# W-Ted/F3D-Gaus

Hardware: AMD Instinct MI355X
Metric: rendered views/sec at 256x256 (N Gaussians, K cams) (higher is better)
Workload: dtype f32; 1 GPU; C2: 1 image/GPU, 196608 Gaussians (sigma0=0.01), 120-view orbit @256x256, GOF forward raster only; timed region = render + 8-bit RGB frames copied to pinned host memory; compositing arithmetic: fast = error-free float32 pairs for the float64 island + hardware exp/rcp/rsq; every channel within 1e-4 of the oracle (RGB <= 3e-7), EXCEPT that the distortion channel (values 1e-7..1e-5 from cancelling fl; gaussians=196608, views=120, resolution=256, tile_cull=1, views_per_call=120, render_mode=fast, channels=all, parallelism=single GPU

## Files before the change

f3d-gaus_amd/csrc/f3dg_api.hip:

```cpp
#include "f3dg_common.h"

#include <stdio.h>
#include <string.h>
#include <time.h>
#include <mutex>
#include <vector>

namespace {

thread_local char g_last_error[512] = "";

size_t align_up(size_t x, size_t a) { return (x + a - 1) / a * a; }

__global__ void init_header_kernel(F3dgHeader* hdr, unsigned capacity, unsigned alpha_fast = 0, unsigned save_aux = 0)
{
    if (threadIdx.x < 64) {
        unsigned* w = reinterpret_cast<unsigned*>(hdr);
        w[threadIdx.x] = 0;
    }
    __syncthreads();
    if (threadIdx.x == 0) { hdr->capacity = capacity; hdr->alpha_fast = alpha_fast; hdr->save_aux = save_aux; }
}

__global__ void fill_background_kernel(int V, size_t HW, const float* __restrict__ bg, int bg_per_view,
                                       float* __restrict__ out)
{
    const size_t n = (size_t)V * F3DG_OUT_CHANNELS * HW;
    for (size_t i = (size_t)blockIdx.x * blockDim.x + threadIdx.x; i < n; i += (size_t)gridDim.x * blockDim.x)
        out[i] = 0.0f;
    (void)bg; (void)bg_per_view;
}

__global__ void export_ids_kernel(const unsigned* __restrict__ src, size_t n, unsigned* __restrict__ dst)
{
    for (size_t i = (size_t)blockIdx.x * blockDim.x + threadIdx.x; i < n; i += (size_t)gridDim.x * blockDim.x)
        dst[i] = src[i] & F3DG_ID_MASK;
}

enum { ST_PREPROCESS = 0, ST_BINNING, ST_RENDER, ST_COUNT };
enum { BW_RENDER = 0, BW_GAUSSIAN, BW_COUNT };
struct ProfCall { hipEvent_t ev[ST_COUNT + 1]; };
struct ProfBwd { hipEvent_t ev[BW_COUNT + 1]; };
struct Prof {
    bool enabled = false;
    std::vector<ProfCall> calls;
    std::vector<ProfCall> pool;
    std::vector<ProfBwd> bwd;
};
thread_local Prof g_prof;

ProfCall* prof_begin(hipStream_t s)
{
    if (!g_prof.enabled) return nullptr;
    ProfCall c;
    if (!g_prof.pool.empty()) { c = g_prof.pool.back(); g_prof.pool.pop_back(); }
    else for (int i = 0; i <= ST_COUNT; i++) if (hipEventCreate(&c.ev[i]) != hipSuccess) return nullptr;
    g_prof.calls.push_back(c);
    (void)hipEventRecord(c.ev[0], s);
    return &g_prof.calls.back();
}
inline void prof_mark(ProfCall* c, int stage_done, hipStream_t s) { if (c) (void)hipEventRecord(c->ev[stage_done + 1], s); }

}

int f3dg_prof_bwd_begin(hipStream_t s)
{
    if (!g_prof.enabled) return -1;
    ProfBwd b;
    for (int i = 0; i <= BW_COUNT; i++) if (hipEventCreate(&b.ev[i]) != hipSuccess) return -1;
    g_prof.bwd.push_back(b);
    (void)hipEventRecord(b.ev[0], s);
    return (int)g_prof.bwd.size() - 1;
}
void f3dg_prof_bwd_mark(int slot, int stage_done, hipStream_t s)
{
    if (slot >= 0 && slot < (int)g_prof.bwd.size()) (void)hipEventRecord(g_prof.bwd[slot].ev[stage_done + 1], s);
}

int g_f3dg_small_path = 1;
int g_f3dg_small_path_aux = 1;
namespace {
struct SmallShape { unsigned v[4]; };
std::vector<SmallShape> g_small_disabled;
std::mutex g_small_mutex, g_sites_mutex;
bool small_disabled(unsigned P, unsigned V, unsigned W, unsigned H)
{
    std::lock_guard<std::mutex> lock(g_small_mutex);
    for (const SmallShape& d : g_small_disabled)
        if (d.v[0] == P && d.v[1] == V && d.v[2] == W && d.v[3] == H) return true;
    return false;
}
void small_disable(unsigned P, unsigned V, unsigned W, unsigned H)
{
    std::lock_guard<std::mutex> lock(g_small_mutex);
    for (const SmallShape& d : g_small_disabled)
        if (d.v[0] == P && d.v[1] == V && d.v[2] == W && d.v[3] == H) return;
    g_small_disabled.push_back({{P, V, W, H}});
}
}
std::atomic<unsigned long long> g_f3dg_kernel_launches{0};
int g_f3dg_render_fast = 1;
int g_f3dg_render_pack = -1;
int g_f3dg_render_count = 0;
int g_f3dg_render_lowocc = 1;
#define F3DG_RENDER_UNROLL_DEFAULT -1
#define F3DG_RENDER_SPLIT_DEFAULT -1
int g_f3dg_render_split = F3DG_RENDER_SPLIT_DEFAULT;
int g_f3dg_render_unroll = F3DG_RENDER_UNROLL_DEFAULT;
int g_f3dg_bwd_occ = 5;
int g_f3dg_tile_cull = 1;
int g_f3dg_reference_kernels = 0;

extern "C" int f3dg_set_option(const char* name, int value)
{
    if (!name) return F3DG_ERR_BAD_ARG;
    if (strcmp(name, "render_fast") == 0) { g_f3dg_render_fast = value < 0 ? 0 : value > 2 ? 2 : value; return F3DG_OK; }
    if (strcmp(name, "tile_cull") == 0) { g_f3dg_tile_cull = value != 0; return F3DG_OK; }
    if (strcmp(name, "small_path") == 0) { g_f3dg_small_path = value != 0; if (value == 2) { std::lock_guard<std::mutex> lock(g_small_mutex); g_small_disabled.clear(); } return F3DG_OK; }
    if (strcmp(name, "small_path_aux") == 0) { g_f3dg_small_path_aux = value != 0; return F3DG_OK; }
    if (strcmp(name, "render_pack") == 0) { g_f3dg_render_pack = value < 0 ? -1 : value != 0; return F3DG_OK; }
    if (strcmp(name, "render_pack_th") == 0) { g_f3dg_render_pack_th = value < 0 ? 0 : value > 64 ? 64 : value; return F3DG_OK; }
    if (strcmp(name, "render_scan") == 0) { g_f3dg_render_scan = value < 0 ? -1 : value != 0; return F3DG_OK; }
    if (strcmp(name, "render_scan_min") == 0) { g_f3dg_render_scan_min = value < 0 ? 0 : value > 64 ? 64 : value; return F3DG_OK; }
    if (strcmp(name, "render_scan_th") == 0) { g_f3dg_render_scan_th = value < 0 ? 0 : value > 64 ? 64 : value; return F3DG_OK; }
    if (strcmp(name, "render_lowocc") == 0) { g_f3dg_render_lowocc = value < 0 ? 1 : value > 64 ? 64 : value; return F3DG_OK; }
    if (strcmp(name, "render_unroll") == 0) { g_f3dg_render_unroll = value < 0 ? F3DG_RENDER_UNROLL_DEFAULT : value < 1 ? 1 : value > 2 ? 2 : value; return F3DG_OK; }
    if (strcmp(name, "bwd_dense") == 0) { g_f3dg_bwd_dense = value != 0; return F3DG_OK; }
    if (strcmp(name, "bwd_occ") == 0) { g_f3dg_bwd_occ = (value >= 2 && value <= 6) ? value : 5; return F3DG_OK; }
    if (strcmp(name, "render_count") == 0) { g_f3dg_render_count = value != 0; return F3DG_OK; }
    if (strcmp(name, "time_launches") == 0) { g_f3dg_time_launches = value != 0; return F3DG_OK; }
    if (strcmp(name, "reference_kernels") == 0) { g_f3dg_reference_kernels = value != 0; return F3DG_OK; }
    if (strcmp(name, "render_split") == 0) { g_f3dg_render_split = value < 1 ? F3DG_RENDER_SPLIT_DEFAULT : value > 3 ? 3 : value; return F3DG_OK; }
    return F3DG_ERR_BAD_ARG;
}

int g_f3dg_time_launches = 0;
namespace { struct LaunchSite { const char* file; int line; long long ns, n, max_ns; }; std::vector<LaunchSite> g_sites; }
long long f3dg_now_ns()
{
    timespec ts;
    clock_gettime(CLOCK_MONOTONIC, &ts);
    return (long long)ts.tv_sec * 1000000000ll + ts.tv_nsec;
}
void f3dg_note_launch_time(const char* file, int line, long long ns)
{
    std::lock_guard<std::mutex> lock(g_sites_mutex);
    for (LaunchSite& s : g_sites)
        if (s.file == file && s.line == line) { s.ns += ns; s.n++; if (ns > s.max_ns) s.max_ns = ns; return; }
    g_sites.push_back({file, line, ns, 1, ns});
}
extern "C" int f3dg_debug_launch_times(int reset)
{
    std::lock_guard<std::mutex> lock(g_sites_mutex);
    for (const LaunchSite& s : g_sites) {
        const char* base = strrchr(s.file, '/');
        fprintf(stderr, "%-22s:%4d  %6lld launches  %8.2f us avg  %9.1f us max\n", base ? base + 1 : s.file, s.line, s.n,
                1e-3 * (double)s.ns / (double)s.n, 1e-3 * (double)s.max_ns);
    }
    if (reset) g_sites.clear();
    return F3DG_OK;
}

extern "C" long long f3dg_debug_launch_count(int reset)
{
    return (long long)(reset ? g_f3dg_kernel_launches.exchange(0ull) : g_f3dg_kernel_launches.load());
}

extern "C" int f3dg_profile_enable(int on)
{
    g_prof.enabled = on != 0;
    return F3DG_OK;
}

extern "C" int f3dg_profile_collect(double* h_stage_ms, int* h_calls) { return f3dg_profile_collect_calls(h_stage_ms, h_calls, nullptr, 0); }

extern "C" int f3dg_profile_collect_calls(double* h_stage_ms, int* h_calls, double* h_per_call, int max_calls)
{
    double sum[ST_COUNT] = { 0, 0, 0 };
    int k = 0;
    for (ProfCall& c : g_prof.calls) {
        F3DG_HIP_CHECK(hipEventSynchronize(c.ev[ST_COUNT]));
        for (int i = 0; i < ST_COUNT; i++) {
            float ms = 0;
            F3DG_HIP_CHECK(hipEventElapsedTime(&ms, c.ev[i], c.ev[i + 1]));
            sum[i] += ms;
            if (h_per_call && k < max_calls) h_per_call[3 * k + i] = ms;
        }
        k++;
        g_prof.pool.push_back(c);
    }
    double bsum[BW_COUNT] = { 0, 0 };
    for (ProfBwd& b : g_prof.bwd) {
        F3DG_HIP_CHECK(hipEventSynchronize(b.ev[BW_COUNT]));
        for (int i = 0; i < BW_COUNT; i++) {
            float ms = 0;
            F3DG_HIP_CHECK(hipEventElapsedTime(&ms, b.ev[i], b.ev[i + 1]));
            bsum[i] += ms;
        }
        for (int i = 0; i <= BW_COUNT; i++) (void)hipEventDestroy(b.ev[i]);
    }
    g_prof.bwd.clear();
    if (h_calls) *h_calls = (int)g_prof.calls.size();
    g_prof.calls.clear();
    if (h_stage_ms) {
        for (int i = 0; i < ST_COUNT; i++) h_stage_ms[i] = sum[i];
        for (int i = 0; i < BW_COUNT; i++) h_stage_ms[ST_COUNT + i] = bsum[i];
    }
    return F3DG_OK;
}

int f3dg_set_hip_error(hipError_t e, const char* where)
{
    snprintf(g_last_error, sizeof g_last_error, "%s: %s", where, hipGetErrorString(e));
    return F3DG_ERR_HIP;
}

extern "C" const char* f3dg_version(void) { return "f3dg-hip gfx950 0.2.0"; }
extern "C" const char* f3dg_last_error(void) { return g_last_error; }

int f3dg_sort_passes(int V, int T);

F3dgLayout f3dg_layout(int P, int W, int H, int V, long long cap)
{
    F3dgLayout L;
    memset(&L, 0, sizeof L);
    const size_t VP = (size_t)V * (size_t)(P > 0 ? P : 1);
    const size_t HW = (size_t)W * H;
    const size_t T = (size_t)((W + F3DG_TILE - 1) / F3DG_TILE) * ((H + F3DG_TILE - 1) / F3DG_TILE);
    const size_t C = (size_t)(cap > 0 ? cap : 1);
    L.sort_blocks = (unsigned)((C + F3DG_SORT_CHUNK - 1) / F3DG_SORT_CHUNK);
    const size_t scan_a = (VP + F3DG_SCAN_CHUNK - 1) / F3DG_SCAN_CHUNK;
    const size_t gsort_blocks = (size_t)V * (((size_t)(P > 0 ? P : 1) + F3DG_SORT_CHUNK - 1) / F3DG_SORT_CHUNK);
    const size_t tile_blocks = (size_t)L.sort_blocks + (size_t)V;
    const size_t hist_blocks = gsort_blocks > tile_blocks ? gsort_blocks : tile_blocks;
    const size_t scan_b = ((size_t)256 * hist_blocks + F3DG_SCAN_CHUNK - 1) / F3DG_SCAN_CHUNK;
    L.scan_tmp_elems = (unsigned)((scan_a > scan_b ? scan_a : scan_b) + 1);

    size_t off = 0;
    auto take = [&](size_t bytes) { size_t o = off; off = align_up(off + bytes, 256); return o; };
    L.header = take(sizeof(F3dgHeader));
    L.rec = take(VP * sizeof(F3dgRec));
    L.means2D = take(VP * sizeof(float2));
    L.bbox = take(VP * sizeof(float4));
    L.cull = take(VP * sizeof(float4));
    L.depths = take(VP * sizeof(float));
    L.conic = take(VP * sizeof(float4));
    L.radii = take(VP * sizeof(int));
    L.tiles = take(VP * sizeof(unsigned));
    L.offsets = take(VP * sizeof(unsigned));
    L.clamped = take(VP);
    L.rects = take(VP * sizeof(uint2));
    L.gsort = take(4 * VP * sizeof(unsigned));
    L.scan_tmp = take((size_t)L.scan_tmp_elems * sizeof(unsigned));
    L.keys[0] = take(C * 8);
    L.keys[1] = take(C * 4);
    L.vals[0] = take(C * 4);
    L.vals[1] = take(C * 4);
    L.segtab_minmax = (unsigned)((size_t)2 * (V + 1) + (size_t)8 * (V / 8 + 2));
    L.segtab = take(((size_t)L.segtab_minmax + (size_t)2 * V + 2 * gsort_blocks) * sizeof(unsigned));
    L.hist = take((size_t)256 * hist_blocks * sizeof(unsigned));
    L.ranges = take((size_t)V * T * sizeof(uint2));
    L.final_T = take((size_t)V * 4 * HW * sizeof(float));
    L.n_contrib = take((size_t)V * 2 * HW * sizeof(unsigned));
    L.bwd_acc = take(VP * 16 * sizeof(double));
    L.small_cap = f3dg_small_shape(P, W, H, V) ? (unsigned)F3DG_SMALL_CAP : 0u;
    L.small_boxes = take(L.small_cap ? (size_t)V * ((P + 63) / 64) * sizeof(uint2) : 0);
    L.small_cnt = take((size_t)V * T * sizeof(unsigned));
    L.small_list = take((size_t)V * T * L.small_cap * sizeof(unsigned));
    L.total = off;
    return L;
}

extern "C" size_t f3dg_workspace_bytes(int P, int W, int H, int n_views, long long max_rendered)
{
    if (P < 0 || W <= 0 || H <= 0 || n_views <= 0 || max_rendered < 0) return 0;
    return f3dg_layout(P, W, H, n_views, max_rendered).total;
}

namespace {

int check_gaussian_args(int P, int D, int M, const float* means3D, const float* shs, const float* colors_precomp,
                        const float* opacities, const float* scales, const float* rotations, const float* cov3D_precomp,
                        const float* view2gaussian_precomp, const float* viewmatrix, const float* projmatrix,
                        const float* cam_pos)
{
    (void)P;
    if (!means3D || !opacities || !viewmatrix || !projmatrix || !cam_pos) return F3DG_ERR_BAD_ARG;
    if ((shs == nullptr) == (colors_precomp == nullptr)) return F3DG_ERR_BAD_ARG;
    const bool have_sr = scales != nullptr && rotations != nullptr;
    if (have_sr == (cov3D_precomp != nullptr)) return F3DG_ERR_BAD_ARG;
    if (!have_sr && view2gaussian_precomp == nullptr) return F3DG_ERR_BAD_ARG;
    if (shs && (M <= 0 || D < 0 || D > 3 || (D + 1) * (D + 1) > M)) return F3DG_ERR_BAD_ARG;
    return F3DG_OK;
}

int run_geometry(hipStream_t s, char* ws, const F3dgLayout& L, int n_views, int views_per_set, int P, int D, int M, int W, int H,
                 const float* means3D, const float* shs, const float* colors_precomp, const float* opacities,
                 const float* scales, float scale_modifier, const float* rotations, const float* cov3D_precomp,
                 const float* view2gaussian_precomp, const float* viewmatrix, const float* projmatrix,
                 const float* cam_pos, float tan_fovx, float tan_fovy, float focal_x, float focal_y, float kernel_size,
                 int* radii_used, int save_aux, int need_box, int tile_cull, ProfCall* prof, F3dgHeaderInit init, int small = 0)
{
    int rc = f3dg_launch_preprocess(s, n_views, views_per_set, P, D, M, means3D, scales, scale_modifier, rotations, opacities, shs,
                                    cov3D_precomp, colors_precomp, view2gaussian_precomp, viewmatrix, projmatrix,
                                    cam_pos, W, H, tan_fovx, tan_fovy, focal_x, focal_y, kernel_size,
                                    reinterpret_cast<F3dgRec*>(ws + L.rec), reinterpret_cast<float2*>(ws + L.means2D),
                                    reinterpret_cast<float*>(ws + L.depths), reinterpret_cast<unsigned*>(ws + L.gsort),
                                    reinterpret_cast<uint2*>(ws + L.rects),
                                    need_box ? reinterpret_cast<float4*>(ws + L.bbox) : nullptr,
                                    reinterpret_cast<float4*>(ws + L.cull),
                                    reinterpret_cast<float4*>(ws + L.conic), radii_used,
                                    reinterpret_cast<unsigned*>(ws + L.tiles),
                                    reinterpret_cast<unsigned char*>(ws + L.clamped), save_aux, tile_cull, init,
                                    small ? reinterpret_cast<uint2*>(ws + L.small_boxes) : nullptr);
    if (rc != F3DG_OK) return rc;
    prof_mark(prof, ST_PREPROCESS, s);
    rc = small ? f3dg_launch_small_bin(s, n_views, P, W, H, L, ws) : f3dg_launch_binning(s, n_views, P, W, H, L, ws, save_aux);
    if (rc != F3DG_OK) return rc;
    prof_mark(prof, ST_BINNING, s);
    return F3DG_OK;
}

}

extern "C" int f3dg_forward_batched(void* stream, void* workspace, size_t workspace_bytes, long long max_rendered,
                                    int n_views, int P, int D, int M,
                                    const float* background, int W, int H,
                                    const float* means3D, const float* shs, const float* colors_precomp,
                                    const float* opacities, const float* scales, float scale_modifier,
                                    const float* rotations, const float* cov3D_precomp,
                                    const float* view2gaussian_precomp,
                                    const float* viewmatrix, const float* projmatrix, const float* cam_pos,
                                    float tan_fovx, float tan_fovy, float kernel_size,
                                    float* out_color, int* radii, unsigned flags)
{
    return f3dg_forward_sets(stream, workspace, workspace_bytes, max_rendered, 1, n_views, P, D, M, background, W, H, means3D, shs,
                             colors_precomp, opacities, scales, scale_modifier, rotations, cov3D_precomp, view2gaussian_precomp,
                             viewmatrix, projmatrix, cam_pos, tan_fovx, tan_fovy, kernel_size, out_color, radii, flags);
}

extern "C" int f3dg_forward_sets(void* stream, void* workspace, size_t workspace_bytes, long long max_rendered,
                                 int n_sets, int views_per_set, int P, int D, int M,
                                 const float* background, int W, int H,
                                 const float* means3D, const float* shs, const float* colors_precomp,
                                 const float* opacities, const float* scales, float scale_modifier,
                                 const float* rotations, const float* cov3D_precomp,
                                 const float* view2gaussian_precomp,
                                 const float* viewmatrix, const float* projmatrix, const float* cam_pos,
                                 float tan_fovx, float tan_fovy, float kernel_size,
                                 float* out_color, int* radii, unsigned flags)
{
    if (n_sets <= 0 || views_per_set <= 0 || (long long)n_sets * views_per_set > 0x7FFFFFF0ll) return F3DG_ERR_BAD_ARG;
    const int n_views = n_sets * views_per_set;
    hipStream_t s = (hipStream_t)stream;
    if (n_views <= 0 || P < 0 || W <= 0 || H <= 0 || max_rendered < 0 || !out_color || !background || !workspace)
        return F3DG_ERR_BAD_ARG;
    if (max_rendered > 0xFFFFFFF0ll || (long long)n_views * P > 0xFFFFFFF0ll || P > (int)F3DG_ID_MASK)
        return F3DG_ERR_BAD_ARG;
    const F3dgLayout L = f3dg_layout(P, W, H, n_views, max_rendered);
    if (workspace_bytes < L.total) return F3DG_ERR_WORKSPACE;
    char* ws = static_cast<char*>(workspace);
    F3dgHeader* hdr = reinterpret_cast<F3dgHeader*>(ws + L.header);
    const size_t HW = (size_t)W * H;

    const int save_aux = (flags & F3DG_FLAG_SAVE_AUX) ? 1 : 0;
    if ((flags & F3DG_FLAG_SETS_AUX) && !save_aux) return F3DG_ERR_BAD_ARG;
    if (n_sets > 1 && ((save_aux && !(flags & F3DG_FLAG_SETS_AUX)) || view2gaussian_precomp != nullptr)) return F3DG_ERR_BAD_ARG;
    const int fast = g_f3dg_reference_kernels || (flags & F3DG_FLAG_EXACT) ? 0 : (flags & F3DG_FLAG_FAST) ? 1 : f3dg_render_uses_fast(save_aux);
    const int tile_cull = (flags & F3DG_FLAG_NO_TILE_CULL) ? 0 : g_f3dg_tile_cull;
    const int small = g_f3dg_small_path && !(flags & F3DG_FLAG_NO_SMALL_PATH) && (!save_aux || g_f3dg_small_path_aux) && n_sets == 1 && P > 0 && L.small_cap != 0 &&
                      !g_f3dg_reference_kernels && !small_disabled((unsigned)P, (unsigned)n_views, (unsigned)W, (unsigned)H);
    const F3dgHeaderInit hinit = { hdr, (unsigned)max_rendered, (unsigned)fast, (unsigned)save_aux, (unsigned)small,
                                   { (unsigned)P, (unsigned)n_views, (unsigned)W, (unsigned)H } };
    if (P == 0)
        F3DG_KLAUNCH(init_header_kernel, dim3(1), dim3(64), 0, s, hdr, (unsigned)max_rendered, (unsigned)fast, (unsigned)save_aux);

    if (P == 0) {
        F3DG_KLAUNCH(fill_background_kernel, dim3(1024), dim3(256), 0, s, n_views, HW, background,
                           (flags & F3DG_FLAG_BG_PER_VIEW) ? 1 : 0, out_color);
        F3DG_HIP_CHECK(hipGetLastError());
        return F3DG_OK;
    }
    int rc = check_gaussian_args(P, D, M, means3D, shs, colors_precomp, opacities, scales, rotations, cov3D_precomp,
                                 view2gaussian_precomp, viewmatrix, projmatrix, cam_pos);
    if (rc != F3DG_OK) return rc;

    const float focal_y = H / (2.0f * tan_fovy);
    const float focal_x = W / (2.0f * tan_fovx);
    int* radii_used = radii ? radii : reinterpret_cast<int*>(ws + L.radii);

    ProfCall* prof = prof_begin(s);
    rc = run_geometry(s, ws, L, n_views, views_per_set, P, D, M, W, H, means3D, shs, colors_precomp, opacities, scales, scale_modifier,
                      rotations, cov3D_precomp, view2gaussian_precomp, viewmatrix, projmatrix, cam_pos, tan_fovx,
                      tan_fovy, focal_x, focal_y, kernel_size, radii_used, save_aux,
                      save_aux , tile_cull, prof, hinit, small);
    if (rc != F3DG_OK) return rc;

    rc = f3dg_launch_render(s, n_views, P, W, H, focal_x, focal_y, hdr,
                              reinterpret_cast<const uint2*>(ws + L.ranges),
                              reinterpret_cast<const unsigned*>(ws + (small ? L.small_list : L.vals[0])),
                              reinterpret_cast<const F3dgRec*>(ws + L.rec),
                              reinterpret_cast<const float4*>(ws + L.cull), background,
                              (flags & F3DG_FLAG_BG_PER_VIEW) ? 1 : 0, out_color,
                              reinterpret_cast<float*>(ws + L.final_T),
                              reinterpret_cast<unsigned*>(ws + L.n_contrib), save_aux,
                              flags & (F3DG_FLAG_SKIP_NORMAL | F3DG_FLAG_SKIP_DISTORTION), fast, (flags & F3DG_FLAG_SCAN) ? 1 : 0);
    prof_mark(prof, ST_RENDER, s);
    return rc;
}

extern "C" size_t f3dg_integrate_workspace_bytes(int P, int PN, int W, int H, long long max_rendered)
{
    if (P < 0 || PN < 0 || W <= 0 || H <= 0 || max_rendered < 0) return 0;
    return f3dg_integ_layout(P, PN, W, H, max_rendered).total;
}

extern "C" size_t f3dg_integrate_workspace_bytes_batched(int P, int PN, int W, int H, int n_views, long long max_rendered)
{
    if (P < 0 || PN < 0 || W <= 0 || H <= 0 || n_views <= 0 || max_rendered < 0) return 0;
    return f3dg_integ_layout(P, PN, W, H, max_rendered, n_views).total;
}

extern "C" long long f3dg_integrate_prepare_batched(void* stream, void* workspace, size_t workspace_bytes, long long max_rendered,
                                                    int n_views, int PN_max, int P, int D, int M, const float* background, int W, int H,
                                                    const float* means3D, const float* shs, const float* colors_precomp,
                                                    const float* opacities, const float* scales, float scale_modifier,
                                                    const float* rotations, const float* cov3D_precomp,
                                                    const float* view2gaussian_precomp, const float* viewmatrix,
                                                    const float* projmatrix, const float* cam_pos, float tan_fovx, float tan_fovy,
                                                    float kernel_size, float* out_color, int* radii, long long* h_needed)
{
    hipStream_t s = (hipStream_t)stream;
    if (n_views <= 0 || PN_max < 0 || P <= 0 || W <= 0 || H <= 0 || max_rendered < 0 || !out_color || !workspace || !background)
        return F3DG_ERR_BAD_ARG;
    if (max_rendered > 0xFFFFFFF0ll || (long long)n_views * P > 0xFFFFFFF0ll || P > (int)F3DG_ID_MASK) return F3DG_ERR_BAD_ARG;
    const F3dgLayout L = f3dg_layout(P, W, H, n_views, max_rendered);
    const F3dgIntegLayout I = f3dg_integ_layout(P, PN_max, W, H, max_rendered, n_views);
    if (workspace_bytes < I.total) return F3DG_ERR_WORKSPACE;
    char* ws = static_cast<char*>(workspace);
    F3dgHeader* hdr = reinterpret_cast<F3dgHeader*>(ws + L.header);
    if (h_needed) *h_needed = 0;
    const F3dgHeaderInit hinit = { hdr, (unsigned)max_rendered, 0u, 0u, 0u, { (unsigned)P, (unsigned)n_views, (unsigned)W, (unsigned)H } };
    int rc = check_gaussian_args(P, D, M, means3D, shs, colors_precomp, opacities, scales, rotations, cov3D_precomp,
                                 view2gaussian_precomp, viewmatrix, projmatrix, cam_pos);
    if (rc != F3DG_OK) return rc;
    const float focal_y = H / (2.0f * tan_fovy);
    const float focal_x = W / (2.0f * tan_fovx);
    int* radii_used = radii ? radii : reinterpret_cast<int*>(ws + L.radii);
    rc = run_geometry(s, ws, L, n_views, n_views, P, D, M, W, H, means3D, shs, colors_precomp, opacities, scales, scale_modifier,
                      rotations, cov3D_precomp, view2gaussian_precomp, viewmatrix, projmatrix, cam_pos, tan_fovx,
                      tan_fovy, focal_x, focal_y, kernel_size, radii_used, 0, 1 ,
                      0 , nullptr, hinit);
    if (rc != F3DG_OK) return rc;
    rc = f3dg_launch_integrate_pass1(s, n_views, P, W, H, focal_x, focal_y, L, I, ws, background, out_color);
    if (rc != F3DG_OK) return rc;
    long long n = 0;
    rc = f3dg_read_status(stream, workspace, &n);
    if (h_needed) *h_needed = n;
    if (rc != F3DG_OK) return rc;
    return n;
}

extern "C" long long f3dg_integrate_prepare(void* stream, void* workspace, size_t workspace_bytes, long long max_rendered,
                                            int PN_max, int P, int D, int M, const float* background, int W, int H,
                                            const float* means3D, const float* shs, const float* colors_precomp,
                                            const float* opacities, const float* scales, float scale_modifier,
                                            const float* rotations, const float* cov3D_precomp,
                                            const float* view2gaussian_precomp, const float* viewmatrix,
                                            const float* projmatrix, const float* cam_pos, float tan_fovx, float tan_fovy,
                                            float kernel_size, float* out_color, int* radii, long long* h_needed)
{
    return f3dg_integrate_prepare_batched(stream, workspace, workspace_bytes, max_rendered, 1, PN_max, P, D, M, background, W, H, means3D,
                                          shs, colors_precomp, opacities, scales, scale_modifier, rotations, cov3D_precomp,
                                          view2gaussian_precomp, viewmatrix, projmatrix, cam_pos, tan_fovx, tan_fovy, kernel_size,
                                          out_color, radii, h_needed);
}

extern "C" int f3dg_integrate_points_view(void* stream, void* workspace, size_t workspace_bytes, long long max_rendered,
                                          int n_views, int view, int PN, int P, int W, int H, const float* points3D,
                                          const float* viewmatrix, float tan_fovx, float tan_fovy, float* out_color,
                                          float* out_alpha_integrated, float* out_color_integrated, float* alpha_min)
{
    hipStream_t s = (hipStream_t)stream;
    if (PN < 0 || P <= 0 || W <= 0 || H <= 0 || max_rendered < 0 || !out_color || !workspace || !viewmatrix || n_views <= 0 ||
        view < 0 || view >= n_views)
        return F3DG_ERR_BAD_ARG;
    if (PN == 0) return F3DG_OK;
    if (!points3D) return F3DG_ERR_BAD_ARG;
    const F3dgLayout L = f3dg_layout(P, W, H, n_views, max_rendered);
    const F3dgIntegLayout I = f3dg_integ_layout(P, PN, W, H, max_rendered, n_views);
    if (workspace_bytes < I.total) return F3DG_ERR_WORKSPACE;
    const float focal_y = H / (2.0f * tan_fovy);
    const float focal_x = W / (2.0f * tan_fovx);
    return f3dg_launch_integrate_points(s, view, P, PN, W, H, focal_x, focal_y, L, I, static_cast<char*>(workspace), points3D,
                                        viewmatrix, out_color, out_alpha_integrated, out_color_integrated, alpha_min);
}

extern "C" int f3dg_debug_integrate_redo(void* stream, const void* workspace, int P, int PN_max, int W, int H, int n_views,
                                         long long max_rendered, int* h_tiles)
{
    if (!workspace || !h_tiles || P <= 0 || W <= 0 || H <= 0 || n_views <= 0 || PN_max < 0 || max_rendered < 0) return F3DG_ERR_BAD_ARG;
    const F3dgIntegLayout I = f3dg_integ_layout(P, PN_max, W, H, max_rendered, n_views);
    const size_t T = (size_t)((W + F3DG_TILE - 1) / F3DG_TILE) * ((H + F3DG_TILE - 1) / F3DG_TILE);
    std::vector<unsigned> flags((size_t)n_views * T);
    F3DG_HIP_CHECK(hipMemcpyAsync(flags.data(), static_cast<const char*>(workspace) + I.redo, flags.size() * sizeof(unsigned),
                                  hipMemcpyDeviceToHost, (hipStream_t)stream));
    F3DG_HIP_CHECK(hipStreamSynchronize((hipStream_t)stream));
    int n = 0;
    for (unsigned f : flags) n += f != 0u;
    *h_tiles = n;
    return F3DG_OK;
}

extern "C" int f3dg_integrate_points(void* stream, void* workspace, size_t workspace_bytes, long long max_rendered,
                                     int PN, int P, int W, int H, const float* points3D, const float* viewmatrix,
                                     float tan_fovx, float tan_fovy, float* out_color, float* out_alpha_integrated,
                                     float* out_color_integrated, float* alpha_min)
{
    return f3dg_integrate_points_view(stream, workspace, workspace_bytes, max_rendered, 1, 0, PN, P, W, H, points3D, viewmatrix, tan_fovx,
                                      tan_fovy, out_color, out_alpha_integrated, out_color_integrated, alpha_min);
}

extern "C" long long f3dg_integrate(void* stream, void* workspace, size_t workspace_bytes, long long max_rendered,
                                    int PN, int P, int D, int M, const float* background, int W, int H,
                                    const float* points3D, const float* means3D, const float* shs,
                                    const float* colors_precomp, const float* opacities, const float* scales,
                                    float scale_modifier, const float* rotations, const float* cov3D_precomp,
                                    const float* view2gaussian_precomp, const float* viewmatrix,
                                    const float* projmatrix, const float* cam_pos, float tan_fovx, float tan_fovy,
                                    float kernel_size, const float* subpixel_offset, int prefiltered,
                                    float* out_color, int* radii, float* out_alpha_integrated,
                                    float* out_color_integrated, long long* h_needed)
{
    (void)subpixel_offset;
    (void)prefiltered;
    hipStream_t s = (hipStream_t)stream;
    if (PN < 0 || P < 0 || W <= 0 || H <= 0 || max_rendered < 0 || !out_color || !workspace) return F3DG_ERR_BAD_ARG;
    if (PN > 0 && (!points3D || !out_alpha_integrated || !out_color_integrated)) return F3DG_ERR_BAD_ARG;
    if (h_needed) *h_needed = 0;
    if (P == 0 || PN == 0) {
        if (workspace_bytes < sizeof(F3dgHeader)) return F3DG_ERR_WORKSPACE;
        F3DG_KLAUNCH(init_header_kernel, dim3(1), dim3(64), 0, s, reinterpret_cast<F3dgHeader*>(workspace), (unsigned)max_rendered);
        int rc = f3dg_launch_integrate_fill(s, W, H, PN, out_color, out_alpha_integrated, out_color_integrated);
        if (rc != F3DG_OK) return rc;
        F3DG_HIP_CHECK(hipStreamSynchronize(s));
        return 0;
    }
    const long long n = f3dg_integrate_prepare(stream, workspace, workspace_bytes, max_rendered, PN, P, D, M, background, W, H,
                                               means3D, shs, colors_precomp, opacities, scales, scale_modifier, rotations,
                                               cov3D_precomp, view2gaussian_precomp, viewmatrix, projmatrix, cam_pos,
                                               tan_fovx, tan_fovy, kernel_size, out_color, radii, h_needed);
    if (n < 0) return n;
    const int rc = f3dg_integrate_points(stream, workspace, workspace_bytes, max_rendered, PN, P, W, H, points3D, viewmatrix,
                                         tan_fovx, tan_fovy, out_color, out_alpha_integrated, out_color_integrated, nullptr);
    if (rc != F3DG_OK) return rc;
    return n;
}

extern "C" int f3dg_read_status(void* stream, const void* workspace, long long* h_num_rendered)
{
    if (!workspace) return F3DG_ERR_BAD_ARG;
    F3dgHeader h;
    F3DG_HIP_CHECK(hipMemcpyAsync(&h, workspace, sizeof h, hipMemcpyDeviceToHost, (hipStream_t)stream));
    F3DG_HIP_CHECK(hipStreamSynchronize((hipStream_t)stream));
    if (h_num_rendered) *h_num_rendered = (long long)h.num_rendered;
    if (h.small_overflow) small_disable(h.small_shape[0], h.small_shape[1], h.small_shape[2], h.small_shape[3]);
    return h.overflow ? F3DG_ERR_OVERFLOW : F3DG_OK;
}

namespace {
struct StatusSlot { F3dgHeader* host; hipEvent_t ev; bool busy; };
std::vector<StatusSlot> g_status;
std::mutex g_status_mutex;
int finish_status(const F3dgHeader& h, long long* h_num_rendered)
{
    if (h_num_rendered) *h_num_rendered = (long long)h.num_rendered;
    if (h.small_overflow) small_disable(h.small_shape[0], h.small_shape[1], h.small_shape[2], h.small_shape[3]);
    return h.overflow ? F3DG_ERR_OVERFLOW : F3DG_OK;
}
}

extern "C" int f3dg_status_post(void* stream, const void* workspace)
{
    if (!workspace) return F3DG_ERR_BAD_ARG;
    int ticket = -1;
    StatusSlot sl = { nullptr, nullptr, false };
    {
        std::lock_guard<std::mutex> lock(g_status_mutex);
        for (size_t i = 0; i < g_status.size(); i++)
            if (!g_status[i].busy) { ticket = (int)i; break; }
        if (ticket < 0) {
            StatusSlot fresh = { nullptr, nullptr, false };
            F3DG_HIP_CHECK(hipHostMalloc(reinterpret_cast<void**>(&fresh.host), sizeof(F3dgHeader), hipHostMallocDefault));
            const hipError_t e = hipEventCreateWithFlags(&fresh.ev, hipEventDisableTiming);
            if (e != hipSuccess) { (void)hipHostFree(fresh.host); return f3dg_set_hip_error(e, "hipEventCreateWithFlags"); }
            g_status.push_back(fresh);
            ticket = (int)g_status.size() - 1;
        }
        g_status[ticket].busy = true;
        sl = g_status[ticket];
    }
    hipError_t e = hipMemcpyAsync(sl.host, workspace, sizeof(F3dgHeader), hipMemcpyDeviceToHost, (hipStream_t)stream);
    if (e == hipSuccess) e = hipEventRecord(sl.ev, (hipStream_t)stream);
    if (e != hipSuccess) {
        std::lock_guard<std::mutex> lock(g_status_mutex);
        g_status[ticket].busy = false;
        return f3dg_set_hip_error(e, "f3dg_status_post");
    }
    return ticket;
}

extern "C" int f3dg_status_poll(int ticket, int wait, long long* h_num_rendered)
{
    StatusSlot sl;
    {
        std::lock_guard<std::mutex> lock(g_status_mutex);
        if (ticket < 0 || ticket >= (int)g_status.size() || !g_status[ticket].busy) return F3DG_ERR_BAD_ARG;
        sl = g_status[ticket];
    }
    if (wait) F3DG_HIP_CHECK(hipEventSynchronize(sl.ev));
    else {
        const hipError_t q = hipEventQuery(sl.ev);
        if (q == hipErrorNotReady) return F3DG_PENDING;
        F3DG_HIP_CHECK(q);
    }
    const int rc = finish_status(*sl.host, h_num_rendered);
    std::lock_guard<std::mutex> lock(g_status_mutex);
    g_status[ticket].busy = false;
    return rc;
}

extern "C" int f3dg_backward_pairs(void* stream, const void* workspace, long long* h_pairs)
{
    if (!workspace || !h_pairs) return F3DG_ERR_BAD_ARG;
    F3dgHeader h;
    F3DG_HIP_CHECK(hipMemcpyAsync(&h, workspace, sizeof h, hipMemcpyDeviceToHost, (hipStream_t)stream));
    F3DG_HIP_CHECK(hipStreamSynchronize((hipStream_t)stream));
    *h_pairs = (long long)h.bwd_pairs;
    return h.bwd_stale ? F3DG_ERR_STATE : F3DG_OK;
}

extern "C" long long f3dg_forward(void* stream, void* workspace, size_t workspace_bytes, long long max_rendered,
                                  int P, int D, int M, const float* background, int W, int H,
                                  const float* means3D, const float* shs, const float* colors_precomp,
                                  const float* opacities, const float* scales, float scale_modifier,
                                  const float* rotations, const float* cov3D_precomp,
                                  const float* view2gaussian_precomp,
                                  const float* viewmatrix, const float* projmatrix, const float* cam_pos,
                                  float tan_fovx, float tan_fovy, float kernel_size, int prefiltered,
                                  float* out_color, int* radii, unsigned flags, long long* h_needed)
{
    (void)prefiltered;
    int rc = f3dg_forward_batched(stream, workspace, workspace_bytes, max_rendered, 1, P, D, M, background, W, H,
                                  means3D, shs, colors_precomp, opacities, scales, scale_modifier, rotations,
                                  cov3D_precomp, view2gaussian_precomp, viewmatrix, projmatrix, cam_pos, tan_fovx,
                                  tan_fovy, kernel_size, out_color, radii, flags & ~F3DG_FLAG_BG_PER_VIEW);
    if (rc != F3DG_OK) return rc;
    long long n = 0;
    rc = f3dg_read_status(stream, workspace, &n);
    if (h_needed) *h_needed = n;
    if (rc != F3DG_OK) return rc;
    return n;
}

extern "C" int f3dg_debug_export(void* stream, const void* workspace, int P, int W, int H, int n_views,
                                 long long max_rendered, float* rec , float* means2D ,
                                 float* conic , unsigned* tiles , unsigned* offsets ,
                                 unsigned char* clamped , unsigned long long* keys_sorted ,
                                 unsigned* point_list , unsigned* ranges ,
                                 float* final_T , unsigned* n_contrib , float* depths )
{
    hipStream_t s = (hipStream_t)stream;
    if (!workspace) return F3DG_ERR_BAD_ARG;
    const F3dgLayout L = f3dg_layout(P, W, H, n_views, max_rendered);
    const char* ws = static_cast<const char*>(workspace);
    const size_t VP = (size_t)n_views * P, HW = (size_t)W * H;
    F3dgHeader h;
    F3DG_HIP_CHECK(hipMemcpyAsync(&h, ws + L.header, sizeof h, hipMemcpyDeviceToHost, s));
    F3DG_HIP_CHECK(hipStreamSynchronize(s));
    if ((means2D || conic || tiles || offsets || clamped || keys_sorted || final_T || n_contrib || depths) && !h.save_aux)
        return F3DG_ERR_BAD_ARG;
    if (h.small_path) {
        if (h.overflow) return F3DG_ERR_OVERFLOW;
        if (offsets || keys_sorted) return F3DG_ERR_STATE;
        const int rcs = f3dg_launch_small_export(s, n_views, W, H, L, ws, point_list, ranges);
        if (rcs != F3DG_OK) return rcs;
        point_list = nullptr;
        ranges = nullptr;
    }
    const size_t T = (size_t)((W + F3DG_TILE - 1) / F3DG_TILE) * ((H + F3DG_TILE - 1) / F3DG_TILE);
    const size_t C = (size_t)max_rendered;
    if (keys_sorted && P > 0) {
        const int rck = f3dg_launch_export_keys(s, n_views, P, W, H, L, const_cast<char*>(ws));
        if (rck != F3DG_OK) return rck;
    }
#define CP(dst, off, bytes) if (dst && (bytes)) F3DG_HIP_CHECK(hipMemcpyAsync(dst, ws + (off), (bytes), hipMemcpyDeviceToDevice, s))
    CP(rec, L.rec, VP * sizeof(F3dgRec));
    CP(means2D, L.means2D, VP * 8);
    CP(conic, L.conic, VP * 16);
    CP(tiles, L.tiles, VP * 4);
    CP(offsets, L.offsets, VP * 4);
    CP(clamped, L.clamped, VP);
    CP(keys_sorted, L.keys[0], C * 8);
    if (point_list && C)
        F3DG_KLAUNCH(export_ids_kernel, dim3((unsigned)((C + 1023) / 1024 < 4096 ? (C + 1023) / 1024 : 4096)), dim3(256), 0, s,
                           reinterpret_cast<const unsigned*>(ws + L.vals[0]), C, point_list);
    CP(ranges, L.ranges, (size_t)n_views * T * 8);
    CP(final_T, L.final_T, (size_t)n_views * 4 * HW * 4);
    CP(n_contrib, L.n_contrib, (size_t)n_views * 2 * HW * 4);
    CP(depths, L.depths, VP * 4);
#undef CP
    return F3DG_OK;
}
```

f3d-gaus_amd/csrc/f3dg_binning.hip:

```cpp
#include "f3dg_common.h"

namespace {

typedef unsigned long long u64;
typedef unsigned int u32;

__global__ void __launch_bounds__(F3DG_BLOCK)
scan_reduce_kernel(const u32* __restrict__ in, u64 n, u32* __restrict__ block_sums)
{
    __shared__ u32 wsum[F3DG_BLOCK / 64];
    const u64 base = (u64)blockIdx.x * F3DG_SCAN_CHUNK;
    u32 s = 0;
#pragma unroll
    for (int i = 0; i < F3DG_SCAN_ITEMS; i++) {
        const u64 k = base + (u64)i * F3DG_BLOCK + threadIdx.x;
        if (k < n) s += in[k];
    }
#pragma unroll
    for (int off = 32; off > 0; off >>= 1) s += __shfl_down(s, off, 64);
    if ((threadIdx.x & 63) == 0) wsum[threadIdx.x >> 6] = s;
    __syncthreads();
    if (threadIdx.x == 0) block_sums[blockIdx.x] = wsum[0] + wsum[1] + wsum[2] + wsum[3];
}

__global__ void __launch_bounds__(1024)
scan_blocksums_kernel(u32* __restrict__ block_sums, u32 nblocks, F3dgHeader* __restrict__ hdr)
{
    __shared__ u32 wtot[16];
    __shared__ u32 carry_s;
    __shared__ u64 carry64_s, wtot64[16];
    if (threadIdx.x == 0) { carry_s = 0; carry64_s = 0; }
    __syncthreads();
    const int lane = threadIdx.x & 63, wave = threadIdx.x >> 6;
    for (u32 start = 0; start < nblocks; start += 1024) {
        const u32 i = start + threadIdx.x;
        const u32 v = i < nblocks ? block_sums[i] : 0;
        u32 x = v;
#pragma unroll
        for (int off = 1; off < 64; off <<= 1) {
            const u32 y = __shfl_up(x, off, 64);
            if (lane >= off) x += y;
        }
        if (lane == 63) wtot[wave] = x;
        unsigned long long v64 = v;
#pragma unroll
        for (int off = 32; off > 0; off >>= 1) v64 += __shfl_down(v64, off, 64);
        if (lane == 0) wtot64[wave] = v64;
        __syncthreads();
        u32 wave_off = 0;
        for (int w = 0; w < wave; w++) wave_off += wtot[w];
        const u32 carry = carry_s;
        if (i < nblocks) block_sums[i] = carry + wave_off + x - v;
        __syncthreads();
        if (threadIdx.x == 1023) {
            carry_s = carry + wave_off + x;
            u64 t = 0;
            for (int w = 0; w < 16; w++) t += wtot64[w];
            carry64_s += t;
        }
        __syncthreads();
    }
    if (hdr && threadIdx.x == 0) {
        const u64 total = carry64_s;
        hdr->num_rendered = total > 0xFFFFFFFFull ? 0xFFFFFFFFu : (u32)total;
        hdr->overflow = total > (u64)hdr->capacity ? 1u : 0u;
    }
}

__global__ void __launch_bounds__(F3DG_BLOCK)
scan_apply_kernel(const u32* in, u32* out , u64 n, const u32* __restrict__ block_sums,
                  int exclusive)
{
    __shared__ u32 wtot[F3DG_BLOCK / 64];
    const u64 base = (u64)blockIdx.x * F3DG_SCAN_CHUNK + (u64)threadIdx.x * F3DG_SCAN_ITEMS;
    u32 v[F3DG_SCAN_ITEMS];
    u32 s = 0;
    if (base + F3DG_SCAN_ITEMS <= n) {
#pragma unroll
        for (int i = 0; i < F3DG_SCAN_ITEMS / 4; i++) {
            const uint4 w = reinterpret_cast<const uint4*>(in + base)[i];
            v[4 * i] = w.x; v[4 * i + 1] = w.y; v[4 * i + 2] = w.z; v[4 * i + 3] = w.w;
        }
    } else {
#pragma unroll
        for (int i = 0; i < F3DG_SCAN_ITEMS; i++) v[i] = (base + i < n) ? in[base + i] : 0;
    }
#pragma unroll
    for (int i = 0; i < F3DG_SCAN_ITEMS; i++) s += v[i];
    const int lane = threadIdx.x & 63, wave = threadIdx.x >> 6;
    u32 x = s;
#pragma unroll
    for (int off = 1; off < 64; off <<= 1) {
        const u32 y = __shfl_up(x, off, 64);
        if (lane >= off) x += y;
    }
    if (lane == 63) wtot[wave] = x;
    __syncthreads();
    u32 run = block_sums[blockIdx.x] + x - s;
    for (int w = 0; w < wave; w++) run += wtot[w];
    u32 o[F3DG_SCAN_ITEMS];
#pragma unroll
    for (int i = 0; i < F3DG_SCAN_ITEMS; i++) {
        const u32 before = run;
        run += v[i];
        o[i] = exclusive ? before : run;
    }
    if (base + F3DG_SCAN_ITEMS <= n) {
#pragma unroll
        for (int i = 0; i < F3DG_SCAN_ITEMS / 4; i++)
            reinterpret_cast<uint4*>(out + base)[i] = make_uint4(o[4 * i], o[4 * i + 1], o[4 * i + 2], o[4 * i + 3]);
    } else {
#pragma unroll
        for (int i = 0; i < F3DG_SCAN_ITEMS; i++)
            if (base + i < n) out[base + i] = o[i];
    }
}


struct SegChunk {
    u64 seg_base;
    u64 obase;
    u32 n;
    u32 cps;
    u32 c;
    u32 seg;
};

struct SegTable {
    const u32* vstart;
    const u32* bglob;
    const u32* xprefix;
    u32 xstride;
    u32 V;
};

struct ShiftDigit {
    int shift;
    u32 mask = 255u;
    __device__ __forceinline__ u32 operator()(u32 k) const { return (k >> shift) & mask; }
};
struct CompactDigit {
    u32 kbase;
    __device__ __forceinline__ u32 operator()(u32 k) const { const u32 d = (k - kbase) >> 16; return d < 255u ? d : 255u; }
};

template <typename K, typename DIGIT, bool MINMAX = false>
__device__ __forceinline__ void hist_chunk(const K* __restrict__ keys, const SegChunk& ck, const DIGIT digit, u32* __restrict__ hist,
                                           u32 (*h)[256], u32* __restrict__ minmax = nullptr)
{
    u32 kmin = 0xFFFFFFFFu, kmax = 0u;
#pragma unroll
    for (int w = 0; w < F3DG_BLOCK / 64; w++) h[w][threadIdx.x] = 0;
    __syncthreads();
    u32* hw = h[threadIdx.x >> 6];
    constexpr int VEC = 16 / (int)sizeof(K);
    typedef K __attribute__((ext_vector_type(VEC))) KV;
    const u64 base = (u64)ck.c * F3DG_SORT_CHUNK;
    const u64 g0 = ck.seg_base + base;
    const u64 g1 = ck.seg_base + ((u64)ck.n - base < (u64)F3DG_SORT_CHUNK ? (u64)ck.n : base + F3DG_SORT_CHUNK);
    for (u64 a = (g0 & ~(u64)(VEC - 1)) + (u64)threadIdx.x * VEC; a < g1; a += (u64)F3DG_BLOCK * VEC) {
        const KV w = *reinterpret_cast<const KV*>(keys + a);
#pragma unroll
        for (int q = 0; q < VEC; q++) {
            if (a + q >= g0 && a + q < g1) {
                const u32 key = (u32)w[q];
                atomicAdd(&hw[digit(key)], 1u);
                if (MINMAX && key != 0xFFFFFFFFu) { kmin = key < kmin ? key : kmin; kmax = key > kmax ? key : kmax; }
            }
        }
    }
    __shared__ u32 wmm[2][F3DG_BLOCK / 64];
    if (MINMAX) {
#pragma unroll
        for (int off = 32; off > 0; off >>= 1) {
            const u32 a = __shfl_down(kmin, off, 64), b = __shfl_down(kmax, off, 64);
            kmin = a < kmin ? a : kmin; kmax = b > kmax ? b : kmax;
        }
        if ((threadIdx.x & 63) == 0) { wmm[0][threadIdx.x >> 6] = kmin; wmm[1][threadIdx.x >> 6] = kmax; }
    }
    __syncthreads();
    if (MINMAX && threadIdx.x == 0) {
        u32 a = wmm[0][0], b = wmm[1][0];
#pragma unroll
        for (int w = 1; w < F3DG_BLOCK / 64; w++) { a = wmm[0][w] < a ? wmm[0][w] : a; b = wmm[1][w] > b ? wmm[1][w] : b; }
        minmax[0] = a; minmax[1] = b;
    }
    hist[ck.obase + (u64)threadIdx.x * ck.cps + ck.c] = h[0][threadIdx.x] + h[1][threadIdx.x] + h[2][threadIdx.x] + h[3][threadIdx.x];
}

struct ScatterShared {
    u32 cnt[F3DG_BLOCK / 64][256];
    u32 lbase[256];
    u32 gdelta[256];
    u32 wtot[F3DG_BLOCK / 64];
    u32 sval[F3DG_SORT_CHUNK];
};

template <typename K, bool IOTA, typename DIGIT>
__device__ __forceinline__ void scatter_chunk(const K* __restrict__ keys_in, const u32* __restrict__ vals_in, K* __restrict__ keys_out,
                                              u32* __restrict__ vals_out, const SegChunk& ck, const DIGIT digit,
                                              const u32* __restrict__ offsets , ScatterShared& sh, K* skey)
{
    const u32 n = ck.n;
    const u64 block_base = (u64)ck.c * F3DG_SORT_CHUNK;
    const u32 in_block = (u32)((n - block_base) < (u64)F3DG_SORT_CHUNK ? (n - block_base) : (u64)F3DG_SORT_CHUNK);
    const int lane = threadIdx.x & 63, wave = threadIdx.x >> 6;
#pragma unroll
    for (int w = 0; w < F3DG_BLOCK / 64; w++) sh.cnt[w][threadIdx.x] = 0;
    __syncthreads();

    const u64 wave_base = block_base + (u64)wave * (64 * F3DG_SORT_ITEMS);
    u32 key[F3DG_SORT_ITEMS];
    u32 val[F3DG_SORT_ITEMS];
    u32 rank[F3DG_SORT_ITEMS];
    const u64 lane_lt = ((u64)1 << lane) - 1;
#pragma unroll
    for (int r = 0; r < F3DG_SORT_ITEMS; r++) {
        const u64 i = wave_base + (u64)r * 64 + lane;
        const bool valid = i < n;
        key[r] = valid ? (u32)keys_in[ck.seg_base + i] : 0u;
        val[r] = IOTA ? (u32)i : (valid ? vals_in[ck.seg_base + i] : 0u);
    }
#pragma unroll
    for (int r = 0; r < F3DG_SORT_ITEMS; r++) {
        const u64 i = wave_base + (u64)r * 64 + lane;
        const bool valid = i < n;
        const u32 d = digit(key[r]);
        u64 diff = 0;
#pragma unroll
        for (int b = 0; b < 8; b++) {
            const u32 own = (u32)((int)(d << (31 - b)) >> 31);
            const u64 bal = __ballot(own != 0u);
            diff |= bal ^ (((u64)own << 32) | own);
        }
        const u64 same = __ballot(valid) & ~diff;
        const u32 below = (u32)__popcll(same & lane_lt);
        const u32 prev = sh.cnt[wave][d];
        rank[r] = prev + below;
        __builtin_amdgcn_wave_barrier();
        if (valid && below == 0) sh.cnt[wave][d] = prev + (u32)__popcll(same);
        __builtin_amdgcn_wave_barrier();
    }
    __syncthreads();
    {
        const u32 d = threadIdx.x;
        const u32 c0 = sh.cnt[0][d], c1 = sh.cnt[1][d], c2 = sh.cnt[2][d], c3 = sh.cnt[3][d];
        const u32 tot = c0 + c1 + c2 + c3;
        u32 x = tot;
#pragma unroll
        for (int off = 1; off < 64; off <<= 1) {
            const u32 y = __shfl_up(x, off, 64);
            if (lane >= off) x += y;
        }
        if (lane == 63) sh.wtot[wave] = x;
        __syncthreads();
        u32 excl = x - tot;
        for (int w = 0; w < wave; w++) excl += sh.wtot[w];
        sh.lbase[d] = excl;
        sh.gdelta[d] = offsets[ck.obase + (u64)d * ck.cps + ck.c] - excl;
        sh.cnt[0][d] = excl;
        sh.cnt[1][d] = excl + c0;
        sh.cnt[2][d] = excl + c0 + c1;
        sh.cnt[3][d] = excl + c0 + c1 + c2;
    }
    __syncthreads();
#pragma unroll
    for (int r = 0; r < F3DG_SORT_ITEMS; r++) {
        const u64 i = wave_base + (u64)r * 64 + lane;
        if (i < n) {
            const u32 d = digit(key[r]);
            const u32 slot = sh.cnt[wave][d] + rank[r];
            skey[slot] = (K)key[r];
            sh.sval[slot] = val[r];
        }
    }
    __syncthreads();
    for (u32 slot = threadIdx.x; slot < in_block; slot += F3DG_BLOCK) {
        const K k = skey[slot];
        const u32 d = digit((u32)k);
        const u32 pos = sh.gdelta[d] + slot;
        if (keys_out) keys_out[pos] = k;
        vals_out[pos] = sh.sval[slot];
    }
}

__device__ __forceinline__ SegChunk fixed_chunk(u32 seg_len, u32 cps)
{
    u32 seg, c;
    f3dg_xcd_map(blockIdx.x, gridDim.x / cps, cps, seg, c);
    SegChunk ck;
    ck.seg_base = (u64)seg * seg_len; ck.obase = (u64)seg * 256u * cps; ck.n = seg_len; ck.cps = cps; ck.c = c; ck.seg = seg;
    return ck;
}

__device__ __forceinline__ bool gsort_compact(const u32* __restrict__ minmax, u32 view, u32& kbase)
{
    const u32 kmin = minmax[2 * view], kmax = minmax[2 * view + 1];
    kbase = kmin & 0xFFFF0000u;
    return kmin <= kmax && ((kmax - kbase) >> 24) == 0u;
}

template <int PASS>
__global__ void __launch_bounds__(F3DG_BLOCK)
gsort_hist_kernel(const u32* __restrict__ keys, u32 seg_len, u32 cps, u32* __restrict__ hist, const u32* __restrict__ minmax,
                  u32* __restrict__ chunk_minmax)
{
    __shared__ u32 h[F3DG_BLOCK / 64][256];
    const SegChunk ck = fixed_chunk(seg_len, cps);
    if constexpr (PASS == 0) {
        hist_chunk<u32, ShiftDigit>(keys, ck, ShiftDigit{0}, hist, h);
    } else if constexpr (PASS == 1) {
        hist_chunk<u32, ShiftDigit, true>(keys, ck, ShiftDigit{8}, hist, h, chunk_minmax + 2 * ((size_t)ck.seg * cps + ck.c));
    } else {
        u32 kbase;
        const bool compact = gsort_compact(minmax, ck.seg, kbase);
        if (!compact) {
            hist_chunk<u32, ShiftDigit>(keys, ck, ShiftDigit{8 * PASS}, hist, h);
        } else if constexpr (PASS == 2) {
            hist_chunk<u32, CompactDigit>(keys, ck, CompactDigit{kbase}, hist, h);
        } else {
            const u64 base = (u64)ck.c * F3DG_SORT_CHUNK;
            const u32 in_chunk = (u32)((ck.n - base) < (u64)F3DG_SORT_CHUNK ? (ck.n - base) : (u64)F3DG_SORT_CHUNK);
            hist[ck.obase + (u64)threadIdx.x * ck.cps + ck.c] = threadIdx.x == 0 ? in_chunk : 0u;
        }
    }
}

__global__ void __launch_bounds__(1024)
gsort_scan_kernel(u32 n_per_seg , u32 seg_len, u32* __restrict__ hist)
{
    __shared__ u32 wtot[16];
    __shared__ u32 carry_s;
    u32* h = hist + (size_t)blockIdx.x * n_per_seg;
    const u32 lane = threadIdx.x & 63u, wave = threadIdx.x >> 6;
    if (threadIdx.x == 0) carry_s = blockIdx.x * seg_len;
    __syncthreads();
    for (u32 base = 0; base < n_per_seg; base += 4096u) {
        const u32 i = base + 4u * threadIdx.x;
        uint4 v = make_uint4(0u, 0u, 0u, 0u);
        if (i < n_per_seg) v = *reinterpret_cast<const uint4*>(h + i);
        const u32 tot = v.x + v.y + v.z + v.w;
        u32 x = tot;
#pragma unroll
        for (int off = 1; off < 64; off <<= 1) {
            const u32 y = __shfl_up(x, off, 64);
            if (lane >= (u32)off) x += y;
        }
        if (lane == 63u) wtot[wave] = x;
        __syncthreads();
        u32 before = carry_s + x - tot;
        for (u32 w = 0; w < wave; w++) before += wtot[w];
        if (i < n_per_seg)
            *reinterpret_cast<uint4*>(h + i) = make_uint4(before, before + v.x, before + v.x + v.y, before + v.x + v.y + v.z);
        __syncthreads();
        if (threadIdx.x == 1023u) carry_s = before + tot;
        __syncthreads();
    }
}

__global__ void __launch_bounds__(64)
gsort_range_kernel(u32 cps, const u32* __restrict__ chunk_minmax, u32* __restrict__ minmax)
{
    u32 kmin = 0xFFFFFFFFu, kmax = 0u;
    for (u32 c = threadIdx.x; c < cps; c += 64) {
        const u32 a = chunk_minmax[2 * ((size_t)blockIdx.x * cps + c)], b = chunk_minmax[2 * ((size_t)blockIdx.x * cps + c) + 1];
        kmin = a < kmin ? a : kmin; kmax = b > kmax ? b : kmax;
    }
#pragma unroll
    for (int off = 32; off > 0; off >>= 1) {
        const u32 a = __shfl_down(kmin, off, 64), b = __shfl_down(kmax, off, 64);
        kmin = a < kmin ? a : kmin; kmax = b > kmax ? b : kmax;
    }
    if (threadIdx.x == 0) { minmax[2 * blockIdx.x] = kmin; minmax[2 * blockIdx.x + 1] = kmax; }
}

template <int PASS>
__global__ void __launch_bounds__(F3DG_BLOCK)
gsort_scatter_kernel(const u32* __restrict__ keys_in, const u32* __restrict__ vals_in, u32* __restrict__ keys_out,
                     u32* __restrict__ vals_out, u32 seg_len, u32 cps, const u32* __restrict__ offsets, const u32* __restrict__ minmax)
{
    __shared__ ScatterShared sh;
    __shared__ u32 skey[F3DG_SORT_CHUNK];
    const SegChunk ck = fixed_chunk(seg_len, cps);
    if constexpr (PASS == 0) {
        scatter_chunk<u32, true, ShiftDigit>(keys_in, vals_in, keys_out, vals_out, ck, ShiftDigit{0}, offsets, sh, skey);
    } else if constexpr (PASS == 1) {
        scatter_chunk<u32, false, ShiftDigit>(keys_in, vals_in, keys_out, vals_out, ck, ShiftDigit{8}, offsets, sh, skey);
    } else {
        u32 kbase;
        const bool compact = gsort_compact(minmax, ck.seg, kbase);
        if (!compact)
            scatter_chunk<u32, false, ShiftDigit>(keys_in, vals_in, PASS == 3 ? (u32*)nullptr : keys_out, vals_out, ck, ShiftDigit{8 * PASS}, offsets, sh, skey);
        else if constexpr (PASS == 2)
            scatter_chunk<u32, false, CompactDigit>(keys_in, vals_in, (u32*)nullptr, vals_out, ck, CompactDigit{kbase}, offsets, sh, skey);
    }
}

__global__ void __launch_bounds__(512)
view_segments_kernel(int V, int P, const u32* __restrict__ offsets_sorted, const F3dgHeader* __restrict__ hdr, u32* __restrict__ vstart,
                     u32* __restrict__ bglob, u32* __restrict__ xprefix, u32 xstride)
{
    __shared__ u32 carry;
    __shared__ u32 wtot[8];
    const u32 lane = threadIdx.x & 63u, wave = threadIdx.x >> 6;
    const bool dead = hdr->overflow != 0;
    auto start_of = [&](u32 v) -> u32 {
        const u64 i = (u64)v * (u64)P;
        return (dead || i == 0) ? 0u : offsets_sorted[i - 1];
    };
    auto chunks_of = [&](u32 v) -> u32 {
        const u32 n = start_of(v + 1) - start_of(v);
        return (n + F3DG_SORT_CHUNK - 1) / F3DG_SORT_CHUNK;
    };
    if (threadIdx.x == 0) carry = 0;
    __syncthreads();
    for (u32 v0 = 0; v0 < (u32)V; v0 += 512) {
        const u32 v = v0 + threadIdx.x;
        const u32 c = v < (u32)V ? chunks_of(v) : 0u;
        u32 x = c;
#pragma unroll
        for (int off = 1; off < 64; off <<= 1) {
            const u32 y = __shfl_up(x, off, 64);
            if (lane >= (u32)off) x += y;
        }
        if (lane == 63) wtot[wave] = x;
        __syncthreads();
        u32 woff = carry;
        for (u32 w = 0; w < wave; w++) woff += wtot[w];
        if (v < (u32)V) { vstart[v] = start_of(v); bglob[v] = woff + x - c; }
        __syncthreads();
        if (threadIdx.x == 511) carry = woff + x;
        __syncthreads();
    }
    if (threadIdx.x == 0) { vstart[V] = start_of((u32)V); bglob[V] = carry; }
    const u32 nk = ((u32)V > wave) ? ((u32)V - wave + 7u) / 8u : 0u;
    u32 run = 0;
    for (u32 k0 = 0; k0 < nk; k0 += 64) {
        const u32 k = k0 + lane;
        const u32 c = k < nk ? chunks_of(wave + 8u * k) : 0u;
        u32 x = c;
#pragma unroll
        for (int off = 1; off < 64; off <<= 1) {
            const u32 y = __shfl_up(x, off, 64);
            if (lane >= (u32)off) x += y;
        }
        if (k < nk) xprefix[wave * xstride + k] = run + x - c;
        run += __shfl(x, 63, 64);
    }
    if (lane == 0) xprefix[wave * xstride + nk] = run;
}

__global__ void __launch_bounds__(F3DG_BLOCK)
ranges_from_offsets_kernel(u32 V, u32 T, int tile_bits, const u32* __restrict__ bglob, const u32* __restrict__ offsets,
                           const F3dgHeader* __restrict__ hdr, uint2* __restrict__ ranges)
{
    const u32 i = blockIdx.x * F3DG_BLOCK + threadIdx.x;
    if (i >= V * T) return;
    const u32 v = i / T, t = i % T;
    const u32 b0 = bglob[v], cpv = bglob[v + 1] - b0;
    uint2 r = make_uint2(0u, 0u);
    if (cpv != 0u && !hdr->overflow) {
        const u32 d = ((v << tile_bits) | t) & 255u;
        const u32 lo = offsets[256ull * b0 + (u64)d * cpv], hi = offsets[256ull * b0 + (u64)(d + 1u) * cpv];
        if (hi > lo) r = make_uint2(lo, hi);
    }
    ranges[i] = r;
}

__device__ __forceinline__ bool var_chunk(const SegTable& st, u32 f, u32& k, SegChunk& ck)
{
    const u32 x = blockIdx.x & 7u;
    const u32* xp = st.xprefix + x * st.xstride;
    const u32 nk = (st.V > x) ? (st.V - x + 7u) / 8u : 0u;
    while (k < nk && f >= xp[k + 1]) k++;
    if (k >= nk) return false;
    const u32 v = x + 8u * k;
    const u32 s0 = st.vstart[v], b0 = st.bglob[v];
    ck.seg_base = s0; ck.n = st.vstart[v + 1] - s0; ck.cps = st.bglob[v + 1] - b0; ck.obase = 256ull * b0; ck.c = f - xp[k];
    return true;
}

template <typename K>
__global__ void __launch_bounds__(F3DG_BLOCK)
radix2_hist_var_kernel(const K* __restrict__ keys, SegTable st, int shift, u32 mask, u32* __restrict__ hist)
{
    __shared__ u32 h[F3DG_BLOCK / 64][256];
    u32 k = 0;
    SegChunk ck;
    for (u32 f = blockIdx.x >> 3; var_chunk(st, f, k, ck); f += gridDim.x >> 3)
        hist_chunk<K, ShiftDigit>(keys, ck, ShiftDigit{shift, mask}, hist, h);
}

template <typename K>
__global__ void __launch_bounds__(F3DG_BLOCK)
radix2_scatter_var_kernel(const K* __restrict__ keys_in, const u32* __restrict__ vals_in, K* __restrict__ keys_out,
                          u32* __restrict__ vals_out, SegTable st, int shift, u32 mask, const u32* __restrict__ offsets)
{
    __shared__ ScatterShared sh;
    __shared__ K skey[F3DG_SORT_CHUNK];
    u32 k = 0;
    SegChunk ck;
    for (u32 f = blockIdx.x >> 3; var_chunk(st, f, k, ck); f += gridDim.x >> 3) {
        scatter_chunk<K, false, ShiftDigit>(keys_in, vals_in, keys_out, vals_out, ck, ShiftDigit{shift, mask}, offsets, sh, skey);
        __syncthreads();
    }
}

__global__ void __launch_bounds__(F3DG_BLOCK)
gsort_gather_rects_kernel(int P, u32* __restrict__ gv0, u32* __restrict__ gv1, const u32* __restrict__ minmax,
                          const uint2* __restrict__ rects, u32* __restrict__ tiles_sorted, u32* __restrict__ rx)
{
    constexpr int ITEMS = 4;
    unsigned view, chunk;
    const unsigned cpv = (unsigned)((P + F3DG_BLOCK * ITEMS - 1) / (F3DG_BLOCK * ITEMS));
    f3dg_xcd_map(blockIdx.x, gridDim.x / cpv, cpv, view, chunk);
    const size_t vb = (size_t)view * P;
    u32 kbase;
    const bool pass2 = gsort_compact(minmax, view, kbase);
    const u32* perm = pass2 ? gv1 : gv0;
    u32* ry = pass2 ? gv0 : gv1;
    const int k0 = (int)(chunk * F3DG_BLOCK * ITEMS + threadIdx.x);
    u32 id[ITEMS];
    uint2 r[ITEMS];
#pragma unroll
    for (int i = 0; i < ITEMS; i++) { const int k = k0 + i * F3DG_BLOCK; id[i] = k < P ? perm[vb + k] : 0u; }
#pragma unroll
    for (int i = 0; i < ITEMS; i++) { const int k = k0 + i * F3DG_BLOCK; r[i] = k < P ? rects[vb + id[i]] : make_uint2(0u, 0u); }
#pragma unroll
    for (int i = 0; i < ITEMS; i++) {
        const int k = k0 + i * F3DG_BLOCK;
        if (k < P) {
            tiles_sorted[vb + k] = (((r[i].x >> 16) & F3DG_RECT_COORD) - (r[i].x & F3DG_RECT_COORD)) *
                                   (((r[i].y >> 16) & F3DG_RECT_COORD) - (r[i].y & F3DG_RECT_COORD));
            rx[vb + k] = r[i].x;
            ry[vb + k] = r[i].y;
        }
    }
}

#define F3DG_DUP_CAP 3072
template <typename G>
__global__ void __launch_bounds__(F3DG_BLOCK)
duplicate_sorted_kernel(int P, int tile_bits, int grid_x, const u32* __restrict__ gv0, const u32* __restrict__ gv1,
                        const u32* __restrict__ minmax, const u32* __restrict__ rx,
                        const u32* __restrict__ offsets_sorted,
                        const F3dgHeader* __restrict__ hdr, G* __restrict__ kgrp, u32* __restrict__ vals)
{
    __shared__ G sk[F3DG_DUP_CAP];
    __shared__ u32 sv[F3DG_DUP_CAP];
    if (hdr->overflow) return;
    const int k = blockIdx.x * F3DG_BLOCK + threadIdx.x;
    const int v = blockIdx.y;
    u32 kbase;
    const bool pass2 = gsort_compact(minmax, (u32)v, kbase);
    const u32* perm = pass2 ? gv1 : gv0;
    const u32* ry = pass2 ? gv0 : gv1;
    const size_t first = (size_t)v * P + (size_t)blockIdx.x * F3DG_BLOCK;
    const int in_block = min(F3DG_BLOCK, P - (int)(blockIdx.x * F3DG_BLOCK));
    const u32 base = first == 0 ? 0u : offsets_sorted[first - 1];
    const u32 n = offsets_sorted[first + in_block - 1] - base;
    u32 off0 = 0, cnt = 0, x = 0, y = 0, g = 0;
    if (k < P) {
        const size_t pos = (size_t)v * P + k;
        x = rx[pos]; y = ry[pos];
        const u32 rminx = x & F3DG_RECT_COORD, rmaxx = (x >> 16) & F3DG_RECT_COORD, rminy = y & F3DG_RECT_COORD, rmaxy = (y >> 16) & F3DG_RECT_COORD;
        if (rmaxx > rminx && rmaxy > rminy) {
            g = perm[pos];
            off0 = ((pos == 0) ? 0 : offsets_sorted[pos - 1]) - base;
            cnt = (rmaxx - rminx) * (rmaxy - rminy);
        }
    }
    const u32 rminx = x & F3DG_RECT_COORD, rmaxx = (x >> 16) & F3DG_RECT_COORD, rminy = y & F3DG_RECT_COORD, rmaxy = (y >> 16) & F3DG_RECT_COORD;
    const u32 view_base = (u32)v << tile_bits;
    auto halves = [](u32 t, u32 tmin, u32 tmax, u32 word) -> u32 {
        u32 m = 3u;
        if (t == tmin && (word & F3DG_RECT_SKIP_LO)) m &= ~1u;
        if (t + 1u == tmax && (word & F3DG_RECT_SKIP_HI)) m &= ~2u;
        return m;
    };
    for (u32 wb = 0; wb < n; wb += (u32)F3DG_DUP_CAP) {
        const u32 lo = off0 > wb ? off0 : wb;
        const u32 hi = off0 + cnt < wb + (u32)F3DG_DUP_CAP ? off0 + cnt : wb + (u32)F3DG_DUP_CAP;
        if (lo < hi) {
            const u32 w = rmaxx - rminx, j0 = lo - off0;
            u32 ty = rminy + j0 / w, tx = rminx + j0 % w;
            u32 my = halves(ty, rminy, rmaxy, y);
            for (u32 j = lo; j < hi; j++) {
                const u32 mx = halves(tx, rminx, rmaxx, x);
                sk[j - wb] = (G)(view_base | (ty * (u32)grid_x + tx));
                sv[j - wb] = g | ((((my & 1u) ? mx : 0u) | ((my & 2u) ? mx << 2 : 0u)) << F3DG_ID_BITS);
                if (++tx == rmaxx) { tx = rminx; ty++; my = halves(ty, rminy, rmaxy, y); }
            }
        }
        __syncthreads();
        const u32 in_win = n - wb < (u32)F3DG_DUP_CAP ? n - wb : (u32)F3DG_DUP_CAP;
        for (u32 i = threadIdx.x; i < in_win; i += F3DG_BLOCK) {
            kgrp[base + wb + i] = sk[i];
            vals[base + wb + i] = sv[i];
        }
        __syncthreads();
    }
}

__global__ void __launch_bounds__(F3DG_BLOCK)
export_keys_kernel(u32 nseg, int P, int tile_bits, int T, const uint2* __restrict__ ranges, const F3dgHeader* __restrict__ hdr,
                   const u32* __restrict__ point_list, const float* __restrict__ depths, u64* __restrict__ keys_out)
{
    if (hdr->overflow) return;
    for (u32 seg = blockIdx.x; seg < nseg; seg += gridDim.x) {
        const uint2 r = ranges[seg];
        const u32 view = seg / (u32)T, tile = seg % (u32)T;
        const u64 hi = (u64)((view << tile_bits) | tile) << 32;
        for (u32 i = r.x + threadIdx.x; i < r.y; i += F3DG_BLOCK)
            keys_out[i] = hi | (u64)__float_as_uint(depths[(size_t)view * P + (point_list[i] & F3DG_ID_MASK)]);
    }
}

template <typename G>
__global__ void __launch_bounds__(F3DG_BLOCK)
group_bounds_kernel(const G* __restrict__ kgrp, const F3dgHeader* __restrict__ hdr, int tile_bits, int T, u32* __restrict__ ranges)
{
    const u32 L = hdr->overflow ? 0u : hdr->num_rendered;
    const u32 tmask = (1u << tile_bits) - 1u;
    for (u64 base = ((u64)blockIdx.x * F3DG_BLOCK + threadIdx.x) * 8u; base < L; base += (u64)gridDim.x * F3DG_BLOCK * 8u) {
        G v[8];
        if (base + 8 <= L) {
            typedef G __attribute__((ext_vector_type(8))) G8;
            const G8 w = *reinterpret_cast<const G8*>(kgrp + base);
#pragma unroll
            for (int i = 0; i < 8; i++) v[i] = w[i];
        } else {
#pragma unroll
            for (int i = 0; i < 8; i++) v[i] = base + i < L ? kgrp[base + i] : (G)0;
        }
        u32 prev = base > 0 ? (u32)kgrp[base - 1] : 0u;
        const u32 next = base + 8 < L ? (u32)kgrp[base + 8] : 0u;
#pragma unroll
        for (int i = 0; i < 8; i++) {
            const u64 idx = base + i;
            if (idx < L) {
                const u32 cur = (u32)v[i];
                const u32 nxt = i < 7 ? (u32)v[i + 1] : next;
                const u32 seg = (cur >> tile_bits) * (u32)T + (cur & tmask);
                if (idx == 0 || prev != cur) ranges[2u * seg] = (u32)idx;
                if (idx == L - 1 || nxt != cur) ranges[2u * seg + 1u] = (u32)idx + 1u;
                prev = cur;
            }
        }
    }
}

int bits_for(unsigned long long n_values)
{
    int b = 0;
    while (b < 64 && (n_values - 1) >> b) b++;
    return n_values <= 1 ? 0 : b;
}

}

int f3dg_launch_scan_inclusive(hipStream_t s, const unsigned* in, unsigned* out, unsigned long long n,
                               unsigned* tmp, unsigned tmp_elems, int exclusive, F3dgHeader* hdr_total)
{
    if (n == 0) return F3DG_OK;
    const unsigned nblocks = (unsigned)((n + F3DG_SCAN_CHUNK - 1) / F3DG_SCAN_CHUNK);
    if (nblocks > tmp_elems) return F3DG_ERR_WORKSPACE;
    F3DG_KLAUNCH(scan_reduce_kernel, dim3(nblocks), dim3(F3DG_BLOCK), 0, s, in, (u64)n, tmp);
    F3DG_KLAUNCH(scan_blocksums_kernel, dim3(1), dim3(1024), 0, s, tmp, nblocks, hdr_total);
    F3DG_KLAUNCH(scan_apply_kernel, dim3(nblocks), dim3(F3DG_BLOCK), 0, s, in, out, (u64)n, tmp, exclusive);
    F3DG_HIP_CHECK(hipGetLastError());
    return F3DG_OK;
}

int f3dg_tile_bits(int T) { return bits_for((unsigned long long)T); }


int f3dg_sort_passes(int V, int T)
{
    (void)V;
    const int bits = f3dg_tile_bits(T);
    return bits == 0 ? 0 : (bits + 7) / 8;
}

template <typename G>
static int binning_tail(hipStream_t s, int V, int P, int grid_x, int T, int tile_bits, const F3dgLayout& L, char* ws, F3dgHeader* hdr)
{
    int rc = F3DG_OK;
    const size_t VP = (size_t)V * P;
    u32* scan_tmp = reinterpret_cast<u32*>(ws + L.scan_tmp);
    u32* hist = reinterpret_cast<u32*>(ws + L.hist);
    u32* gk[2] = { reinterpret_cast<u32*>(ws + L.gsort), reinterpret_cast<u32*>(ws + L.gsort) + VP };
    u32* gv[2] = { reinterpret_cast<u32*>(ws + L.gsort) + 2 * VP, reinterpret_cast<u32*>(ws + L.gsort) + 3 * VP };
    G* kgrp[2] = { reinterpret_cast<G*>(ws + L.keys[0]), reinterpret_cast<G*>(ws + L.keys[1]) };
    u32* vals[2] = { reinterpret_cast<u32*>(ws + L.vals[0]), reinterpret_cast<u32*>(ws + L.vals[1]) };
    const dim3 pgrid((P + F3DG_BLOCK - 1) / F3DG_BLOCK, V);

    const u32 cps = (u32)((P + F3DG_SORT_CHUNK - 1) / F3DG_SORT_CHUNK);
    const u32 gblocks = (u32)V * cps;
    u32* minmax = reinterpret_cast<u32*>(ws + L.segtab) + L.segtab_minmax;
    u32* chunk_minmax = minmax + 2 * (size_t)V;
    const bool view_scan = cps <= 64;
#define F3DG_GSORT_PASS(PASS, IN, OUT)                                                                                                     \
    F3DG_KLAUNCH((gsort_hist_kernel<PASS>), dim3(gblocks), dim3(F3DG_BLOCK), 0, s, gk[IN], (u32)P, cps, hist, minmax, chunk_minmax); \
    if (view_scan)                                                                                                                         \
        F3DG_KLAUNCH(gsort_scan_kernel, dim3(V), dim3(1024), 0, s, 256u * cps, (u32)P, hist);                                       \
    else {                                                                                                                                 \
        rc = f3dg_launch_scan_inclusive(s, hist, hist, (unsigned long long)256 * gblocks, scan_tmp, L.scan_tmp_elems, 1, nullptr);        \
        if (rc != F3DG_OK) return rc;                                                                                                      \
    }                                                                                                                                      \
    F3DG_KLAUNCH((gsort_scatter_kernel<PASS>), dim3(gblocks), dim3(F3DG_BLOCK), 0, s, gk[IN], gv[IN], gk[OUT], gv[OUT], (u32)P, cps, hist, minmax)
    F3DG_GSORT_PASS(0, 0, 1);
    F3DG_GSORT_PASS(1, 1, 0);
    F3DG_KLAUNCH(gsort_range_kernel, dim3(V), dim3(64), 0, s, cps, chunk_minmax, minmax);
    F3DG_GSORT_PASS(2, 0, 1);
    F3DG_GSORT_PASS(3, 1, 0);
#undef F3DG_GSORT_PASS
    u32* offsets_sorted = gk[1];
    u32* rx = gk[0];

    F3DG_KLAUNCH(gsort_gather_rects_kernel, dim3((unsigned)V * (unsigned)((P + 4 * F3DG_BLOCK - 1) / (4 * F3DG_BLOCK))), dim3(F3DG_BLOCK), 0, s, P, gv[0], gv[1], minmax,
                           reinterpret_cast<const uint2*>(ws + L.rects), offsets_sorted, rx);
    rc = f3dg_launch_scan_inclusive(s, offsets_sorted, offsets_sorted, (unsigned long long)VP, scan_tmp, L.scan_tmp_elems, 0, hdr);
    if (rc != F3DG_OK) return rc;
    const int passes = f3dg_sort_passes(V, T);
    int src = passes & 1;
    F3DG_KLAUNCH((duplicate_sorted_kernel<G>), pgrid, dim3(F3DG_BLOCK), 0, s, P, tile_bits, grid_x, gv[0], gv[1], minmax, rx, offsets_sorted, hdr,
                       kgrp[src], vals[src]);

    if (passes > 0) {
        SegTable st;
        u32* segtab = reinterpret_cast<u32*>(ws + L.segtab);
        const u32 xstride = (u32)V / 8u + 2u;
        st.vstart = segtab; st.bglob = segtab + (V + 1); st.xprefix = segtab + 2 * (V + 1); st.xstride = xstride; st.V = (u32)V;
        F3DG_KLAUNCH(view_segments_kernel, dim3(1), dim3(512), 0, s, V, P, offsets_sorted, hdr, segtab, segtab + (V + 1),
                           segtab + 2 * (V + 1), xstride);
        const size_t nbmax = (size_t)L.sort_blocks + (size_t)V;
        const u32 per_xcd = (u32)((nbmax + 7) / 8 < 160 ? (nbmax + 7) / 8 : 160);
        const u32 per_xcd_h = (u32)((nbmax + 7) / 8 < 512 ? (nbmax + 7) / 8 : 512);
        const int split = passes == 2 ? (tile_bits + 1) / 2 : 8;
        for (int p = 0; p < passes; p++) {
            const int shift = split * p;
            const u32 mask = passes == 2 ? (1u << (p == 0 ? split : tile_bits - split)) - 1u : 255u;
            F3DG_HIP_CHECK(hipMemsetAsync(hist, 0, sizeof(u32) * 256 * nbmax, s));
            F3DG_KLAUNCH((radix2_hist_var_kernel<G>), dim3(8 * per_xcd_h), dim3(F3DG_BLOCK), 0, s, kgrp[src], st, shift, mask, hist);
            rc = f3dg_launch_scan_inclusive(s, hist, hist, (unsigned long long)256 * nbmax, scan_tmp, L.scan_tmp_elems, 1, nullptr);
            if (rc != F3DG_OK) return rc;
            F3DG_KLAUNCH((radix2_scatter_var_kernel<G>), dim3(8 * per_xcd), dim3(F3DG_BLOCK), 0, s, kgrp[src], vals[src],
                               passes == 1 ? (G*)nullptr : kgrp[src ^ 1], vals[src ^ 1], st, shift, mask, hist);
            src ^= 1;
        }
        if (passes == 1) {
            const u32 nseg = (u32)V * (u32)T;
            F3DG_KLAUNCH(ranges_from_offsets_kernel, dim3((nseg + F3DG_BLOCK - 1) / F3DG_BLOCK), dim3(F3DG_BLOCK), 0, s, (u32)V, (u32)T, tile_bits,
                               segtab + (V + 1), hist, hdr, reinterpret_cast<uint2*>(ws + L.ranges));
            F3DG_HIP_CHECK(hipGetLastError());
            return F3DG_OK;
        }
    }
    F3DG_HIP_CHECK(hipMemsetAsync(ws + L.ranges, 0, sizeof(uint2) * (size_t)V * T, s));
    F3DG_KLAUNCH((group_bounds_kernel<G>), dim3(2048), dim3(F3DG_BLOCK), 0, s, kgrp[0], hdr, tile_bits, T, reinterpret_cast<u32*>(ws + L.ranges));
    F3DG_HIP_CHECK(hipGetLastError());
    return F3DG_OK;
}

int f3dg_launch_binning(hipStream_t s, int V, int P, int W, int H, const F3dgLayout& L, char* ws, int export_offsets)
{
    const int grid_x = (W + F3DG_TILE - 1) / F3DG_TILE, grid_y = (H + F3DG_TILE - 1) / F3DG_TILE;
    const int T = grid_x * grid_y;
    const int tile_bits = f3dg_tile_bits(T);
    F3dgHeader* hdr = reinterpret_cast<F3dgHeader*>(ws + L.header);

    int rc = F3DG_OK;
    if (export_offsets) {
        rc = f3dg_launch_scan_inclusive(s, reinterpret_cast<const u32*>(ws + L.tiles), reinterpret_cast<u32*>(ws + L.offsets),
                                        (unsigned long long)V * P, reinterpret_cast<u32*>(ws + L.scan_tmp), L.scan_tmp_elems, 0, nullptr);
        if (rc != F3DG_OK) return rc;
    }
    const bool small = (((unsigned long long)(V > 0 ? V - 1 : 0) << tile_bits) | ((1ull << tile_bits) - 1ull)) <= 0xFFFFull;
    rc = small ? binning_tail<unsigned short>(s, V, P, grid_x, T, tile_bits, L, ws, hdr)
               : binning_tail<u32>(s, V, P, grid_x, T, tile_bits, L, ws, hdr);
    if (rc != F3DG_OK) return rc;
    F3DG_HIP_CHECK(hipGetLastError());
    return F3DG_OK;
}

int f3dg_launch_export_keys(hipStream_t s, int V, int P, int W, int H, const F3dgLayout& L, char* ws)
{
    const int grid_x = (W + F3DG_TILE - 1) / F3DG_TILE, grid_y = (H + F3DG_TILE - 1) / F3DG_TILE;
    const int T = grid_x * grid_y;
    const u32 nseg = (u32)V * (u32)T;
    const u32 rg = nseg < 65535u * 4u ? nseg : 65535u * 4u;
    F3DG_KLAUNCH(export_keys_kernel, dim3(rg), dim3(F3DG_BLOCK), 0, s, nseg, P, f3dg_tile_bits(T), T,
                       reinterpret_cast<const uint2*>(ws + L.ranges), reinterpret_cast<const F3dgHeader*>(ws + L.header),
                       reinterpret_cast<const u32*>(ws + L.vals[0]), reinterpret_cast<const float*>(ws + L.depths),
                       reinterpret_cast<u64*>(ws + L.keys[0]));
    F3DG_HIP_CHECK(hipGetLastError());
    return F3DG_OK;
}
```

f3d-gaus_amd/csrc/f3dg_common.h:

```cpp
#pragma once
#include <hip/hip_runtime.h>
#include <stddef.h>
#include <stdint.h>

#include "../../include/f3dg.h"

#define F3DG_BLOCK 256
#define F3DG_REC_FLOATS 16
#define F3DG_NEAR_PLANE 0.2
#define F3DG_FAR_PLANE 100.0
#define F3DG_SORT_ITEMS 16
#define F3DG_SORT_CHUNK (F3DG_BLOCK * F3DG_SORT_ITEMS)
#define F3DG_SCAN_ITEMS 16
#define F3DG_SCAN_CHUNK (F3DG_BLOCK * F3DG_SCAN_ITEMS)

#define F3DG_ID_BITS 28
#define F3DG_ID_MASK 0x0FFFFFFFu
#define F3DG_RECT_COORD 0x7FFFu
#define F3DG_RECT_SKIP_LO 0x8000u
#define F3DG_RECT_SKIP_HI 0x80000000u

__device__ __forceinline__ void f3dg_xcd_map(unsigned b, unsigned V, unsigned U, unsigned& view, unsigned& unit)
{
    const unsigned full = (V & ~7u) * U;
    if (b < full) {
        const unsigned slot = b >> 3;
        view = (slot / U) * 8u + (b & 7u);
        unit = slot % U;
    } else {
        const unsigned r = b - full;
        view = (V & ~7u) + r / U;
        unit = r % U;
    }
}

struct F3dgHeader {
    unsigned int num_rendered;
    unsigned int overflow;
    unsigned int capacity;
    unsigned int bwd_stale;
    unsigned int reserved1[2];
    unsigned int alpha_fast;
    unsigned int save_aux;
    unsigned long long bwd_pairs;
    unsigned int small_path;
    unsigned int small_overflow;
    unsigned int small_shape[4];
    unsigned int reserved[48];
};

struct __attribute__((aligned(16))) F3dgRec { float f[F3DG_REC_FLOATS]; };

__device__ __forceinline__ void f3dg_fast_t_G(float aaf, float bhalf, float CC, float& t, float& G)
{
    const float r = __builtin_amdgcn_rcpf(aaf);
    t = -bhalf * r;
    const float p = bhalf * bhalf;
    const float e = fmaf(bhalf, bhalf, -p);
    const float q1 = p * r;
    const float q2 = (fmaf(-q1, aaf, p) + e) * r;
    const float min_value = (CC - q1) - q2;
    G = __builtin_amdgcn_exp2f(fminf(min_value * -0.7213475204444817f, 0.0f));
}

struct F3dgLayout {
    size_t header;
    size_t rec;
    size_t means2D;
    size_t depths;
    size_t bbox;
    size_t cull;
    size_t conic;
    size_t radii;
    size_t tiles;
    size_t offsets;
    size_t clamped;
    size_t rects;
    size_t gsort;
    size_t scan_tmp;
    size_t keys[2];
    size_t vals[2];
    size_t segtab;
    size_t hist;
    size_t ranges;
    size_t final_T;
    size_t n_contrib;
    size_t bwd_acc;
    size_t small_boxes;
    size_t small_cnt;
    size_t small_list;
    unsigned int small_cap;
    size_t total;
    unsigned int sort_blocks;
    unsigned int scan_tmp_elems;
    unsigned int segtab_minmax;
};

F3dgLayout f3dg_layout(int P, int W, int H, int V, long long cap);

struct F3dgIntegLayout {
    size_t pix_points;
    size_t tile_last;
    size_t clear_bytes;
    size_t contrib_n;
    size_t contrib_ids;
    size_t pix_start;
    size_t scan_tmp;
    size_t pt_pix, pt_rank, perm;
    size_t redo;
    size_t total;
    unsigned scan_tmp_elems;
};
F3dgIntegLayout f3dg_integ_layout(int P, int PN, int W, int H, long long cap, int V = 1);

#include <atomic>
extern std::atomic<unsigned long long> g_f3dg_kernel_launches;
extern int g_f3dg_time_launches;
void f3dg_note_launch_time(const char* file, int line, long long ns);
long long f3dg_now_ns();
#define F3DG_KLAUNCH(...) do { g_f3dg_kernel_launches.fetch_add(1ull, std::memory_order_relaxed);                                                                   \
        if (g_f3dg_time_launches) { const long long t0_ = f3dg_now_ns(); hipLaunchKernelGGL(__VA_ARGS__);                  \
                                    f3dg_note_launch_time(__FILE__, __LINE__, f3dg_now_ns() - t0_); }                      \
        else hipLaunchKernelGGL(__VA_ARGS__); } while (0)

int f3dg_set_hip_error(hipError_t e, const char* where);
#define F3DG_HIP_CHECK(expr) do { hipError_t _e = (expr); if (_e != hipSuccess) return f3dg_set_hip_error(_e, #expr); } while (0)

struct F3dgViewConsts {
    const float* viewmatrix;
    const float* projmatrix;
    const float* cam_pos;
};

struct F3dgHeaderInit {
    F3dgHeader* hdr;
    unsigned capacity, alpha_fast, save_aux, small_path;
    unsigned shape[4];
};

int f3dg_launch_preprocess(hipStream_t s, int V, int views_per_set, int P, int D, int M, const float* means3D, const float* scales,
                           float scale_modifier, const float* rotations, const float* opacities, const float* shs,
                           const float* cov3D_precomp, const float* colors_precomp, const float* v2g_precomp,
                           const float* viewmatrix, const float* projmatrix, const float* cam_pos, int W, int H,
                           float tan_fovx, float tan_fovy, float focal_x, float focal_y, float kernel_size,
                           F3dgRec* rec, float2* means2D, float* depths, unsigned* sort_keys, uint2* rects, float4* bbox , float4* cull, float4* conic,
                           int* radii, unsigned* tiles, unsigned char* clamped, int save_aux, int tile_cull, F3dgHeaderInit init,
                           uint2* chunk_boxes = nullptr );

#define F3DG_SMALL_CAP 4096
inline bool f3dg_small_shape(int P, int W, int H, int V)
{
    const long long T = (long long)((W + F3DG_TILE - 1) / F3DG_TILE) * ((H + F3DG_TILE - 1) / F3DG_TILE);
    return V >= 1 && V <= 2 && P >= 1 && P <= (1 << 18) && T <= 1024;
}
int f3dg_launch_small_bin(hipStream_t s, int V, int P, int W, int H, const F3dgLayout& L, char* ws);
int f3dg_launch_small_export(hipStream_t s, int V, int W, int H, const F3dgLayout& L, const char* ws, unsigned* point_list, unsigned* ranges);

int f3dg_launch_scan_inclusive(hipStream_t s, const unsigned* in, unsigned* out, unsigned long long n,
                               unsigned* tmp, unsigned tmp_elems, int exclusive,
                               F3dgHeader* hdr_total );

int f3dg_launch_binning(hipStream_t s, int V, int P, int W, int H, const F3dgLayout& L, char* ws, int export_offsets);
int f3dg_launch_export_keys(hipStream_t s, int V, int P, int W, int H, const F3dgLayout& L, char* ws);

extern int g_f3dg_small_path;
extern int g_f3dg_bwd_occ;
extern int g_f3dg_render_unroll;
extern int g_f3dg_reference_kernels;
int f3dg_launch_render_small(hipStream_t s, int V, int P, int W, int H, float focal_x, float focal_y, const F3dgHeader* hdr, const uint2* ranges,
                         const unsigned* point_list, const F3dgRec* rec, const float4* cull, const float* background, int bg_per_view,
                         float* out_color, int fast, int save_aux, float* final_T, unsigned* n_contrib, int unroll, int split, int count);
extern int g_f3dg_render_split;
extern int g_f3dg_render_lowocc;
extern int g_f3dg_render_count;
int f3dg_prof_bwd_begin(hipStream_t s);
void f3dg_prof_bwd_mark(int slot, int stage_done, hipStream_t s);
int f3dg_render_uses_fast(int save_aux);
extern int g_f3dg_render_fast;

int f3dg_launch_render(hipStream_t s, int V, int P, int W, int H, float focal_x, float focal_y,
                       const F3dgHeader* hdr, const uint2* ranges, const unsigned* point_list, const F3dgRec* rec,
                       const float4* cull, const float* background, int bg_per_view, float* out_color,
                       float* final_T, unsigned* n_contrib, int save_aux, unsigned skip_channels = 0u, int fast = -1 ,
                       int scan = 0 );

extern int g_f3dg_render_pack;
extern int g_f3dg_render_pack_th;
int f3dg_launch_render4(hipStream_t s, int V, int P, int W, int H, float focal_x, float focal_y, const F3dgHeader* hdr, const uint2* ranges,
                        const unsigned* point_list, const F3dgRec* rec, const float4* cull, const float* background, int bg_per_view,
                        float* out_color, int fast, unsigned skip_channels, int count, int save_aux = 0, float* final_T = nullptr,
                        unsigned* n_contrib = nullptr);

extern int g_f3dg_render_scan;
extern int g_f3dg_render_scan_min;
extern int g_f3dg_render_scan_th;
int f3dg_launch_render5(hipStream_t s, int V, int P, int W, int H, float focal_x, float focal_y, const F3dgHeader* hdr, const uint2* ranges,
                        const unsigned* point_list, const F3dgRec* rec, const float4* cull, const float* background, int bg_per_view,
                        float* out_color, unsigned skip_channels, int count);

int f3dg_launch_render5_small(hipStream_t s, int V, int P, int W, int H, float focal_x, float focal_y, const F3dgHeader* hdr, const uint2* ranges,
                              const unsigned* point_list, const F3dgRec* rec, const float4* cull, const float* background, int bg_per_view,
                              float* out_color);
extern int g_f3dg_bwd_dense;
int f3dg_launch_render5_bwd(hipStream_t s, int V, int P, int W, int H, int tiles_x, int T, float focal_x, float focal_y, F3dgHeader* hdr,
                            const uint2* ranges, const unsigned* point_list, const unsigned* small_list, const F3dgRec* rec, const float4* cull,
                            const float2* means2D, const float4* conic, const float* background, int bg_per_view, const float* final_T,
                            const unsigned* n_contrib, const float* dL_dpixels, float* dL_dmean2D, float* dL_dopacity, float* dL_dcolors,
                            double* dL_dv2g_acc);

int f3dg_launch_integrate_fill(hipStream_t s, int W, int H, int PN, float* out_color, float* out_alpha_integrated,
                               float* out_color_integrated);
int f3dg_launch_integrate_pass1(hipStream_t s, int V, int P, int W, int H, float focal_x, float focal_y, const F3dgLayout& L,
                                const F3dgIntegLayout& I, char* ws, const float* background, float* out_color);
int f3dg_launch_integrate_points(hipStream_t s, int view, int P, int PN, int W, int H, float focal_x, float focal_y, const F3dgLayout& L,
                                 const F3dgIntegLayout& I, char* ws, const float* points3D, const float* viewmatrix,
                                 float* out_color, float* out_alpha_integrated, float* out_color_integrated, float* alpha_min);
```

f3d-gaus_amd/csrc/f3dg_preprocess.hip:

```cpp
#include "f3dg_common.h"

namespace {

__device__ __constant__ float SH_C0 = 0.28209479177387814f;
__device__ __constant__ float SH_C1 = 0.4886025119029199f;
__device__ __constant__ float SH_C2[5] = { 1.0925484305920792f, -1.0925484305920792f, 0.31539156525252005f,
                                           -1.0925484305920792f, 0.5462742152960396f };
__device__ __constant__ float SH_C3[7] = { -0.5900435899266435f, 2.890611442640554f, -0.4570457994644658f,
                                           0.3731763325901154f, -0.4570457994644658f, 1.445305721320277f,
                                           -0.5900435899266435f };

struct M3 { float m[3][3]; };

__device__ __forceinline__ M3 mul(const M3& a, const M3& b)
{
    M3 r;
#pragma unroll
    for (int c = 0; c < 3; c++)
#pragma unroll
        for (int q = 0; q < 3; q++)
            r.m[c][q] = a.m[0][q] * b.m[c][0] + a.m[1][q] * b.m[c][1] + a.m[2][q] * b.m[c][2];
    return r;
}
__device__ __forceinline__ M3 transpose(const M3& a)
{
    M3 r;
#pragma unroll
    for (int c = 0; c < 3; c++)
#pragma unroll
        for (int q = 0; q < 3; q++)
            r.m[c][q] = a.m[q][c];
    return r;
}

__device__ __forceinline__ M3 quat_to_R(float4 q)
{
    const float r = q.x, x = q.y, y = q.z, z = q.w;
    M3 R;
    R.m[0][0] = 1.f - 2.f * (y * y + z * z); R.m[0][1] = 2.f * (x * y - r * z);       R.m[0][2] = 2.f * (x * z + r * y);
    R.m[1][0] = 2.f * (x * y + r * z);       R.m[1][1] = 1.f - 2.f * (x * x + z * z); R.m[1][2] = 2.f * (y * z - r * x);
    R.m[2][0] = 2.f * (x * z - r * y);       R.m[2][1] = 2.f * (y * z + r * x);       R.m[2][2] = 1.f - 2.f * (x * x + y * y);
    return R;
}

__device__ __forceinline__ float ndc2Pix(float v, int S) { return (float)(((v + 1.0) * S - 1.0) * 0.5); }

__device__ __forceinline__ float pretest_constant(const float* vg, float thr)
{
    if (thr == __builtin_inff()) return __builtin_inff();
    const double K0 = ((double)vg[9] + 2.0 * (double)thr) * (1.0 - 5e-7);
    return K0 > 0.0 ? (float)K0 : 0.0f;
}

struct CullConic { double m00, m01, m02, m11, m12, m22; bool ok; };
__device__ __forceinline__ CullConic cull_conic(const float* vg, float thr, float tan_fovx, float tan_fovy)
{
#pragma clang fp contract(fast)
    CullConic q;
    q.ok = false;
    const double u = 5.9604644775390625e-08;
    const double C = vg[9];
    const double k = -2.0 * (double)thr + 2e-3;
    const double cK = C - k;
    q.m00 = q.m01 = q.m02 = q.m11 = q.m12 = q.m22 = 0.0;
    if (!(cK > 0.0)) return q;
    const double X = tan_fovx, Y = tan_fovy;
    const double A = fabs((double)vg[0]) * X * X + 2.0 * fabs((double)vg[1]) * X * Y + 2.0 * fabs((double)vg[2]) * X +
                     fabs((double)vg[3]) * Y * Y + 2.0 * fabs((double)vg[4]) * Y + fabs((double)vg[5]);
    const double Bn = fabs((double)vg[6]) * X + fabs((double)vg[7]) * Y + fabs((double)vg[8]);
    const double D = 1.1 * u * (6.0 * cK * A + 7.0 * Bn * Bn);
    const double B0 = vg[6], B1 = vg[7], B2 = vg[8];
    q.m00 = cK * vg[0] - B0 * B0; q.m01 = cK * vg[1] - B0 * B1; q.m02 = cK * vg[2] - B0 * B2;
    q.m11 = cK * vg[3] - B1 * B1; q.m12 = cK * vg[4] - B1 * B2; q.m22 = cK * vg[5] - B2 * B2 - D;
    q.ok = true;
    return q;
}
__device__ __forceinline__ float4 conservative_box(const CullConic& q, float thr, bool have_scale, int W, int H,
                                                   float focal_x, float focal_y)
{
#pragma clang fp contract(fast)
    const float4 all = make_float4(-3.0e38f, 3.0e38f, -3.0e38f, 3.0e38f);
    if (!have_scale || !(thr < 3.0e38f)) return all;
    if (!q.ok) return all;
    const double m00 = q.m00, m01 = q.m01, m02 = q.m02, m11 = q.m11, m12 = q.m12, m22 = q.m22;
    const double D00 = m11 * m22 - m12 * m12, D11 = m00 * m22 - m02 * m02, D22 = m00 * m11 - m01 * m01;
    const double D02 = m01 * m12 - m02 * m11, D12 = m01 * m02 - m00 * m12;
    if (!(m00 > 0.0) || !(D22 > 1e-9 * fabs(m00 * m11))) return all;
    const double dx = D02 * D02 - D00 * D22, dy = D12 * D12 - D11 * D22;
    if (!(dx >= 0.0) || !(dy >= 0.0)) return all;
    const double cx = D02 / D22, cy = D12 / D22;
    const double hx = sqrt(dx) / D22 * 1.001 + 0.25 / focal_x, hy = sqrt(dy) / D22 * 1.001 + 0.25 / focal_y;
    const double x0 = (cx - hx) * focal_x + W / 2. - 0.5, x1 = (cx + hx) * focal_x + W / 2. - 0.5;
    const double y0 = (cy - hy) * focal_y + H / 2. - 0.5, y1 = (cy + hy) * focal_y + H / 2. - 0.5;
    if (!(x0 == x0) || !(x1 == x1) || !(y0 == y0) || !(y1 == y1)) return all;
    return make_float4((float)x0 - 1e-3f * (1.0f + fabsf((float)x0)), (float)x1 + 1e-3f * (1.0f + fabsf((float)x1)),
                       (float)y0 - 1e-3f * (1.0f + fabsf((float)y0)), (float)y1 + 1e-3f * (1.0f + fabsf((float)y1)));
}


__device__ __forceinline__ void conservative_ellipse(const CullConic& q, float thr, bool have_scale, int W, int H,
                                                     float focal_x, float focal_y, double ifx, double ify, float4& e, float& ec)
{
#pragma clang fp contract(fast)
    e = make_float4(0.0f, 0.0f, 0.0f, 0.0f);
    ec = 0.0f;
    const float4 never = make_float4(-1.0e9f, -1.0e9f, 1.0e30f, 0.0f);
    if (thr == __builtin_inff()) { e = never; ec = 1.0e30f; return; }
    if (!have_scale || !(thr < 3.0e38f) || !q.ok) return;
    const double m00 = q.m00, m01 = q.m01, m02 = q.m02, m11 = q.m11, m12 = q.m12, m22 = q.m22;
    const double D22 = m00 * m11 - m01 * m01;
    if (!(m00 > 0.0) || !(m11 > 0.0) || !(D22 > 1e-9 * fabs(m00 * m11))) return;
    double inv_D22 = __builtin_amdgcn_rcp(D22);
    inv_D22 = fma(fma(-D22, inv_D22, 1.0), inv_D22, inv_D22);
    const double cx = (m01 * m12 - m02 * m11) * inv_D22, cy = (m01 * m02 - m00 * m12) * inv_D22;
    const double Qc = m22 + m02 * cx + m12 * cy;
    if (!(Qc == Qc) || !(cx == cx) || !(cy == cy)) return;
    if (Qc > 0.0 && Qc < 1.0e300) { e = never; ec = 1.0e30f; return; }
    if (!(Qc < 0.0)) return;
    const double k = -__builtin_amdgcn_rcp(Qc);
    double a = m00 * k * (ifx * ifx), b = 2.0 * m01 * k * (ifx * ify), c = m11 * k * (ify * ify);
    const double det = a * c - 0.25 * b * b, tr = a + c;
    if (!(det > 0.0) || !(tr < 1.0e300)) return;
    const double disc = (double)(sqrtf((float)fmax(0.25 * tr * tr - det, 0.0)) * 1.000001f);
    double lmax = 0.5 * tr + disc;
    if (!(lmax > 0.0) || !(lmax < 1.0e300)) return;
    if (lmax * lmax > 1000.0 * det) {
        const double lmin = det / lmax;
        if (!(lmin > 0.0)) return;
        double vx = 0.5 * b, vy = lmax - a;
        if (fabs(vx) + fabs(vy) < 1e-300 * lmax || a > c) { vx = lmax - c; vy = 0.5 * b; }
        const double n2 = vx * vx + vy * vy;
        if (!(n2 > 0.0)) return;
        const double d = (lmax - 1000.0 * lmin) / n2;
        a -= d * vx * vx; b -= 2.0 * d * vx * vy; c -= d * vy * vy;
        lmax = 1000.0 * lmin;
        if (!(a > 0.0) || !(c > 0.0) || !(a * c - 0.25 * b * b > 0.0)) return;
    }
    const double s = 1.001 + 0.05 * (double)(sqrtf((float)lmax) * 1.000001f);
    const double px = cx * focal_x + W / 2. - 0.5, py = cy * focal_y + H / 2. - 0.5;
    if (!(fabs(px) < 8192.0) || !(fabs(py) < 8192.0)) return;
    const double is2 = __builtin_amdgcn_rcp(s * s) * (1.0 - 1e-7);
    const float fa = (float)(a * is2), fb = (float)(b * is2), fc = (float)(c * is2);
    if (!(fa > 1.0e-30f) || !(fc > 1.0e-30f) || !(fa < 1.0e30f) || !(fc < 1.0e30f)) return;
    e = make_float4((float)px, (float)py, fa, fb);
    ec = fc;
}

template <bool SAVE_AUX>
__global__ void __launch_bounds__(F3DG_BLOCK)
preprocess_kernel(int P, int D, int M, int views_per_set,
                  const float* __restrict__ means3D, const float* __restrict__ scales, float scale_modifier,
                  const float* __restrict__ rotations, const float* __restrict__ opacities,
                  const float* __restrict__ shs, const float* __restrict__ cov3D_precomp,
                  const float* __restrict__ colors_precomp, const float* __restrict__ v2g_precomp,
                  const float* __restrict__ viewmatrices, const float* __restrict__ projmatrices,
                  const float* __restrict__ cam_positions, int W, int H, int grid_x, int grid_y,
                  float tan_fovx, float tan_fovy, float focal_x, float focal_y, float kernel_size,
                  F3dgRec* __restrict__ rec, float2* __restrict__ means2D, float* __restrict__ depths_out,
                  unsigned* __restrict__ sort_keys, uint2* __restrict__ rects,
                  float4* __restrict__ bbox_out, float4* __restrict__ cull_out,
                  float4* __restrict__ conic_out,
                  int* __restrict__ radii, unsigned* __restrict__ tiles_touched,
                  unsigned char* __restrict__ clamped, int tile_cull,
                  double inv_focal_x, double inv_focal_y, F3dgHeaderInit init, uint2* __restrict__ chunk_boxes)
{
    if (init.hdr != nullptr && blockIdx.x == 0 && blockIdx.y == 0 && threadIdx.x < 64) {
        reinterpret_cast<unsigned*>(init.hdr)[threadIdx.x] = 0;
        if (threadIdx.x == 0) {
            init.hdr->capacity = init.capacity; init.hdr->alpha_fast = init.alpha_fast; init.hdr->save_aux = init.save_aux;
            init.hdr->small_path = init.small_path;
            init.hdr->small_shape[0] = init.shape[0]; init.hdr->small_shape[1] = init.shape[1];
            init.hdr->small_shape[2] = init.shape[2]; init.hdr->small_shape[3] = init.shape[3];
        }
    }
    const int g = blockIdx.x * F3DG_BLOCK + threadIdx.x;
    const int v = blockIdx.y;
    const size_t gs = (size_t)(v / views_per_set) * P + g;
    if (g >= P)
        return;
    const size_t idx = (size_t)v * P + g;
    const float* view = viewmatrices + 16 * v;
    const float* proj = projmatrices + 16 * v;

    int my_radii = 0;
    unsigned my_tiles = 0;
    float4 r0 = make_float4(0, 0, 0, 0), r1 = r0, r2 = r0, r3 = r0;
    float2 xy = make_float2(0, 0);
    float4 con = make_float4(0, 0, 0, 0);
    float4 box = make_float4(-3.0e38f, 3.0e38f, -3.0e38f, 3.0e38f);
    float4 ce = make_float4(-1.0e9f, -1.0e9f, 1.0e30f, 0.0f);
    float cec = 1.0e30f;
    unsigned char clamp_bits = 0;
    float depth = 0.0f;
    uint2 rect = make_uint2(0u, 0u);

    const float px_ = means3D[3 * gs], py_ = means3D[3 * gs + 1], pz_ = means3D[3 * gs + 2];

    const float pvx = view[0] * px_ + view[4] * py_ + view[8] * pz_ + view[12];
    const float pvy = view[1] * px_ + view[5] * py_ + view[9] * pz_ + view[13];
    const float pvz = view[2] * px_ + view[6] * py_ + view[10] * pz_ + view[14];

    if (!(pvz <= 0.2f)) {
        const float hx = proj[0] * px_ + proj[4] * py_ + proj[8] * pz_ + proj[12];
        const float hy = proj[1] * px_ + proj[5] * py_ + proj[9] * pz_ + proj[13];
        const float hw = proj[3] * px_ + proj[7] * py_ + proj[11] * pz_ + proj[15];
        const float p_w = 1.0f / (hw + 0.0000001f);
        const float projx = hx * p_w, projy = hy * p_w;

        float3 scale = make_float3(0, 0, 0);
        float4 rot = make_float4(1, 0, 0, 0);
        if (scales) scale = make_float3(scales[3 * gs], scales[3 * gs + 1], scales[3 * gs + 2]);
        if (rotations) rot = reinterpret_cast<const float4*>(rotations)[gs];

        float c3[6];
        if (cov3D_precomp) {
#pragma unroll
            for (int i = 0; i < 6; i++) c3[i] = cov3D_precomp[6 * gs + i];
        } else {
            M3 S = {};
            S.m[0][0] = scale_modifier * scale.x;
            S.m[1][1] = scale_modifier * scale.y;
            S.m[2][2] = scale_modifier * scale.z;
            const M3 R = quat_to_R(rot);
            const M3 Mm = mul(S, R);
            const M3 Sigma = mul(transpose(Mm), Mm);
            c3[0] = Sigma.m[0][0]; c3[1] = Sigma.m[0][1]; c3[2] = Sigma.m[0][2];
            c3[3] = Sigma.m[1][1]; c3[4] = Sigma.m[1][2]; c3[5] = Sigma.m[2][2];
        }

        float tx = pvx, ty = pvy;
        const float tz = pvz;
        const float limx = 1.3f * tan_fovx;
        const float limy = 1.3f * tan_fovy;
        const float txtz = tx / tz;
        const float tytz = ty / tz;
        tx = fminf(limx, fmaxf(-limx, txtz)) * tz;
        ty = fminf(limy, fmaxf(-limy, tytz)) * tz;

        M3 J;
        J.m[0][0] = focal_x / tz; J.m[0][1] = 0.0f;         J.m[0][2] = -(focal_x * tx) / (tz * tz);
        J.m[1][0] = 0.0f;         J.m[1][1] = focal_y / tz; J.m[1][2] = -(focal_y * ty) / (tz * tz);
        J.m[2][0] = 0.0f;         J.m[2][1] = 0.0f;         J.m[2][2] = 0.0f;
        M3 Wm;
        Wm.m[0][0] = view[0]; Wm.m[0][1] = view[4]; Wm.m[0][2] = view[8];
        Wm.m[1][0] = view[1]; Wm.m[1][1] = view[5]; Wm.m[1][2] = view[9];
        Wm.m[2][0] = view[2]; Wm.m[2][1] = view[6]; Wm.m[2][2] = view[10];
        const M3 T = mul(Wm, J);
        M3 Vrk;
        Vrk.m[0][0] = c3[0]; Vrk.m[0][1] = c3[1]; Vrk.m[0][2] = c3[2];
        Vrk.m[1][0] = c3[1]; Vrk.m[1][1] = c3[3]; Vrk.m[1][2] = c3[4];
        Vrk.m[2][0] = c3[2]; Vrk.m[2][1] = c3[4]; Vrk.m[2][2] = c3[5];
        const M3 cov = mul(mul(transpose(T), transpose(Vrk)), T);

        const float det_0 = (float)fmax(1e-6, (double)(cov.m[0][0] * cov.m[1][1] - cov.m[0][1] * cov.m[0][1]));
        const float det_1 = (float)fmax(1e-6, (double)((cov.m[0][0] + kernel_size) * (cov.m[1][1] + kernel_size) - cov.m[0][1] * cov.m[0][1]));
        float coef = (float)sqrt(det_0 / (det_1 + 1e-6) + 1e-6);
        if (det_0 <= 1e-6 || det_1 <= 1e-6)
            coef = 0.0f;
        const float cx = cov.m[0][0] + kernel_size;
        const float cy = cov.m[0][1];
        const float cz = cov.m[1][1] + kernel_size;

        const float det = (cx * cz - cy * cy);
        if (det != 0.0f) {
            float conic_x = 0.0f, conic_y = 0.0f, conic_z = 0.0f;
            if (SAVE_AUX) {
                const float det_inv = 1.f / det;
                conic_x = cz * det_inv; conic_y = -cy * det_inv; conic_z = cx * det_inv;
            }
            const float mid = 0.5f * (cx + cz);
            const float lambda1 = mid + sqrtf(fmaxf(0.1f, mid * mid - det));
            const float lambda2 = mid - sqrtf(fmaxf(0.1f, mid * mid - det));
            const float my_radius = ceilf(3.f * sqrtf(fmaxf(lambda1, lambda2)));
            const float pix_x = ndc2Pix(projx, W), pix_y = ndc2Pix(projy, H);
            const int max_radius = (int)my_radius;
            const int rminx = min(grid_x, max(0, (int)((pix_x - max_radius) / F3DG_TILE)));
            const int rminy = min(grid_y, max(0, (int)((pix_y - max_radius) / F3DG_TILE)));
            const int rmaxx = min(grid_x, max(0, (int)((pix_x + max_radius + F3DG_TILE - 1) / F3DG_TILE)));
            const int rmaxy = min(grid_y, max(0, (int)((pix_y + max_radius + F3DG_TILE - 1) / F3DG_TILE)));
            const int area = (rmaxx - rminx) * (rmaxy - rminy);
            if (area != 0) {
                float cr, cg, cb;
                if (colors_precomp) {
                    cr = colors_precomp[3 * gs]; cg = colors_precomp[3 * gs + 1]; cb = colors_precomp[3 * gs + 2];
                } else {
                    const float* campos = cam_positions + 3 * v;
                    float dx = px_ - campos[0], dy = py_ - campos[1], dz = pz_ - campos[2];
                    const float len = sqrtf(dx * dx + dy * dy + dz * dz);
                    dx = dx / len; dy = dy / len; dz = dz / len;
                    const float* sh = shs + gs * M * 3;
                    float res[3];
#pragma unroll
                    for (int ch = 0; ch < 3; ch++) res[ch] = SH_C0 * sh[ch];
                    if (D > 0) {
                        const float x = dx, y = dy, z = dz;
#pragma unroll
                        for (int ch = 0; ch < 3; ch++)
                            res[ch] = res[ch] - SH_C1 * y * sh[3 + ch] + SH_C1 * z * sh[6 + ch] - SH_C1 * x * sh[9 + ch];
                        if (D > 1) {
                            const float xx = x * x, yy = y * y, zz = z * z;
                            const float xy_ = x * y, yz = y * z, xz = x * z;
#pragma unroll
                            for (int ch = 0; ch < 3; ch++)
                                res[ch] = res[ch] +
                                    SH_C2[0] * xy_ * sh[12 + ch] +
                                    SH_C2[1] * yz * sh[15 + ch] +
                                    SH_C2[2] * (2.0f * zz - xx - yy) * sh[18 + ch] +
                                    SH_C2[3] * xz * sh[21 + ch] +
                                    SH_C2[4] * (xx - yy) * sh[24 + ch];
                            if (D > 2) {
#pragma unroll
                                for (int ch = 0; ch < 3; ch++)
                                    res[ch] = res[ch] +
                                        SH_C3[0] * y * (3.0f * xx - yy) * sh[27 + ch] +
                                        SH_C3[1] * xy_ * z * sh[30 + ch] +
                                        SH_C3[2] * y * (4.0f * zz - xx - yy) * sh[33 + ch] +
                                        SH_C3[3] * z * (2.0f * zz - 3.0f * xx - 3.0f * yy) * sh[36 + ch] +
                                        SH_C3[4] * x * (4.0f * zz - xx - yy) * sh[39 + ch] +
                                        SH_C3[5] * z * (xx - yy) * sh[42 + ch] +
                                        SH_C3[6] * x * (xx - 3.0f * yy) * sh[45 + ch];
                            }
                        }
                    }
#pragma unroll
                    for (int ch = 0; ch < 3; ch++) {
                        res[ch] += 0.5f;
                        if (res[ch] < 0) clamp_bits |= (unsigned char)(1u << ch);
                        res[ch] = fmaxf(res[ch], 0.0f);
                    }
                    cr = res[0]; cg = res[1]; cb = res[2];
                }

                float vg[10];
                if (v2g_precomp) {
#pragma unroll
                    for (int i = 0; i < 10; i++) vg[i] = v2g_precomp[idx * 10 + i];
                } else {
                    const M3 R = quat_to_R(rot);
                    float G2V[4][3];
#pragma unroll
                    for (int c = 0; c < 3; c++) {
                        const float b0 = R.m[0][c], b1 = R.m[1][c], b2 = R.m[2][c];
#pragma unroll
                        for (int q = 0; q < 3; q++)
                            G2V[c][q] = view[q] * b0 + view[4 + q] * b1 + view[8 + q] * b2 + view[12 + q] * 0.0f;
                    }
#pragma unroll
                    for (int q = 0; q < 3; q++)
                        G2V[3][q] = view[q] * px_ + view[4 + q] * py_ + view[8 + q] * pz_ + view[12 + q] * 1.0f;

                    M3 Rt;
#pragma unroll
                    for (int c = 0; c < 3; c++) {
                        Rt.m[c][0] = G2V[0][c]; Rt.m[c][1] = G2V[1][c]; Rt.m[c][2] = G2V[2][c];
                    }
                    const float t_x = G2V[3][0], t_y = G2V[3][1], t_z = G2V[3][2];
                    const float t2x = (-Rt.m[0][0]) * t_x + (-Rt.m[1][0]) * t_y + (-Rt.m[2][0]) * t_z;
                    const float t2y = (-Rt.m[0][1]) * t_x + (-Rt.m[1][1]) * t_y + (-Rt.m[2][1]) * t_z;
                    const float t2z = (-Rt.m[0][2]) * t_x + (-Rt.m[1][2]) * t_y + (-Rt.m[2][2]) * t_z;

                    const double Sx = 1.0f / ((double)scale.x * scale.x + 1e-7);
                    const double Sy = 1.0f / ((double)scale.y * scale.y + 1e-7);
                    const double Sz = 1.0f / ((double)scale.z * scale.z + 1e-7);
                    const double Cc = t2x * t2x * Sx + t2y * t2y * Sy + t2z * t2z * Sz;

                    M3 SR;
                    SR.m[0][0] = (float)(Sx * Rt.m[0][0]); SR.m[0][1] = (float)(Sy * Rt.m[0][1]); SR.m[0][2] = (float)(Sz * Rt.m[0][2]);
                    SR.m[1][0] = (float)(Sx * Rt.m[1][0]); SR.m[1][1] = (float)(Sy * Rt.m[1][1]); SR.m[1][2] = (float)(Sz * Rt.m[1][2]);
                    SR.m[2][0] = (float)(Sx * Rt.m[2][0]); SR.m[2][1] = (float)(Sy * Rt.m[2][1]); SR.m[2][2] = (float)(Sz * Rt.m[2][2]);

                    const float Bx = SR.m[0][0] * t2x + SR.m[0][1] * t2y + SR.m[0][2] * t2z;
                    const float By = SR.m[1][0] * t2x + SR.m[1][1] * t2y + SR.m[1][2] * t2z;
                    const float Bz = SR.m[2][0] * t2x + SR.m[2][1] * t2y + SR.m[2][2] * t2z;
                    const M3 Sig = mul(transpose(Rt), SR);
                    vg[0] = Sig.m[0][0]; vg[1] = Sig.m[0][1]; vg[2] = Sig.m[0][2];
                    vg[3] = Sig.m[1][1]; vg[4] = Sig.m[1][2]; vg[5] = Sig.m[2][2];
                    vg[6] = Bx; vg[7] = By; vg[8] = Bz; vg[9] = (float)Cc;
                }

                const float opac = opacities[gs] * coef;
                my_radii = max_radius;
                my_tiles = (unsigned)area;
                rect = make_uint2((unsigned)rminx | ((unsigned)rmaxx << 16), (unsigned)rminy | ((unsigned)rmaxy << 16));
                xy = make_float2(pix_x, pix_y);
                con = make_float4(conic_x, conic_y, conic_z, opac);
                r0 = make_float4(vg[0], vg[1], vg[2], vg[3]);
                r1 = make_float4(vg[4], vg[5], vg[6], vg[7]);
                const float thr = opac > 0.0f ? -0.6931471805599453f * __builtin_amdgcn_logf(255.0f * opac) - 1e-4f : (opac <= 0.0f ? __builtin_inff() : opac);
                const float Kpre = pretest_constant(vg, thr);
                {
                    const bool have_scale = scales != nullptr && v2g_precomp == nullptr;
                    CullConic cq;
                    cq.ok = false;
                    if (have_scale && thr < 3.0e38f)
                        cq = cull_conic(vg, thr, tan_fovx, tan_fovy);
                    if (bbox_out)
                        box = conservative_box(cq, thr, have_scale, W, H, focal_x, focal_y);
                    conservative_ellipse(cq, thr, have_scale, W, H, focal_x, focal_y, inv_focal_x, inv_focal_y, ce, cec);
                }
                {
                    const float edet = fmaf(ce.z, cec, -0.25f * ce.w * ce.w);
                    if (edet > 0.0f) {
                        const float iedet = __builtin_amdgcn_rcpf(edet);
                        const float hx = __builtin_amdgcn_sqrtf(cec * iedet) * 1.0005f + 2e-3f, hy = __builtin_amdgcn_sqrtf(ce.z * iedet) * 1.0005f + 2e-3f;
                        int fminx = rminx, fmaxx = rmaxx, fminy = rminy, fmaxy = rmaxy;
                        if (tile_cull) {
                            const float inv_tile = 1.0f / (float)F3DG_TILE;
                            const float lx = ceilf((ce.x - hx - (float)(F3DG_TILE - 1)) * inv_tile), ux = floorf((ce.x + hx) * inv_tile) + 1.0f;
                            const float ly = ceilf((ce.y - hy - (float)(F3DG_TILE - 1)) * inv_tile), uy = floorf((ce.y + hy) * inv_tile) + 1.0f;
                            const int cminx = max(rminx, (int)fminf(fmaxf(lx, 0.0f), (float)grid_x));
                            const int cmaxx = min(rmaxx, (int)fminf(fmaxf(ux, 0.0f), (float)grid_x));
                            const int cminy = max(rminy, (int)fminf(fmaxf(ly, 0.0f), (float)grid_y));
                            const int cmaxy = min(rmaxy, (int)fminf(fmaxf(uy, 0.0f), (float)grid_y));
                            if (cmaxx > cminx && cmaxy > cminy) {
                                my_tiles = (unsigned)((cmaxx - cminx) * (cmaxy - cminy));
                                rect = make_uint2((unsigned)cminx | ((unsigned)cmaxx << 16), (unsigned)cminy | ((unsigned)cmaxy << 16));
                                fminx = cminx; fmaxx = cmaxx; fminy = cminy; fmaxy = cmaxy;
                            } else {
                                my_tiles = 0;
                                rect = make_uint2(0u, 0u);
                            }
                        }
                        if (my_tiles != 0) {
                            if (ce.x - hx > (float)(F3DG_TILE * fminx + 7)) rect.x |= F3DG_RECT_SKIP_LO;
                            if (ce.x + hx < (float)(F3DG_TILE * (fmaxx - 1) + 8)) rect.x |= F3DG_RECT_SKIP_HI;
                            if (ce.y - hy > (float)(F3DG_TILE * fminy + 7)) rect.y |= F3DG_RECT_SKIP_LO;
                            if (ce.y + hy < (float)(F3DG_TILE * (fmaxy - 1) + 8)) rect.y |= F3DG_RECT_SKIP_HI;
                        }
                    }
                }
                r2 = make_float4(vg[8], vg[9], opac, Kpre);
                r3 = make_float4(cr, cg, cb, 0.0f);
                depth = pvz;
            }
        }
    }

    radii[idx] = my_radii;
    rects[idx] = rect;
    if (chunk_boxes) {
        uint2 bx = make_uint2(F3DG_RECT_COORD << 16, F3DG_RECT_COORD << 16);
        if (__ballot(true) == ~0ull) {
            const bool vis = ((rect.x >> 16) & F3DG_RECT_COORD) > (rect.x & F3DG_RECT_COORD) && ((rect.y >> 16) & F3DG_RECT_COORD) > (rect.y & F3DG_RECT_COORD);
            const unsigned mnx = __reduce_min_sync(~0ull, vis ? rect.x & F3DG_RECT_COORD : F3DG_RECT_COORD);
            const unsigned mxx = __reduce_max_sync(~0ull, vis ? (rect.x >> 16) & F3DG_RECT_COORD : 0u);
            const unsigned mny = __reduce_min_sync(~0ull, vis ? rect.y & F3DG_RECT_COORD : F3DG_RECT_COORD);
            const unsigned mxy = __reduce_max_sync(~0ull, vis ? (rect.y >> 16) & F3DG_RECT_COORD : 0u);
            bx = make_uint2(mnx | (mxx << 16), mny | (mxy << 16));
        }
        if ((threadIdx.x & 63u) == 0u) chunk_boxes[(size_t)v * ((P + 63) / 64) + (g >> 6)] = bx;
    }
    sort_keys[idx] = my_tiles ? __float_as_uint(depth) : 0xFFFFFFFFu;
    if (bbox_out) bbox_out[idx] = box;
    if (SAVE_AUX || my_tiles != 0u) {
        r3.w = cec;
        float4* dst = reinterpret_cast<float4*>(rec + idx);
        cull_out[idx] = ce;
        dst[0] = r0; dst[1] = r1; dst[2] = r2; dst[3] = r3;
    }
    if (SAVE_AUX) {
        tiles_touched[idx] = my_tiles;
        means2D[idx] = xy;
        depths_out[idx] = depth;
        conic_out[idx] = con;
        clamped[idx] = clamp_bits;
    }
}

__global__ void mark_visible_kernel(int P, const float* __restrict__ means3D, const float* __restrict__ view,
                                    unsigned char* __restrict__ present)
{
    const int g = blockIdx.x * blockDim.x + threadIdx.x;
    if (g >= P) return;
    const float x = means3D[3 * (size_t)g], y = means3D[3 * (size_t)g + 1], z = means3D[3 * (size_t)g + 2];
    const float pvz = view[2] * x + view[6] * y + view[10] * z + view[14];
    present[g] = !(pvz <= 0.2f);
}

}

int f3dg_launch_preprocess(hipStream_t s, int V, int views_per_set, int P, int D, int M, const float* means3D, const float* scales,
                           float scale_modifier, const float* rotations, const float* opacities, const float* shs,
                           const float* cov3D_precomp, const float* colors_precomp, const float* v2g_precomp,
                           const float* viewmatrix, const float* projmatrix, const float* cam_pos, int W, int H,
                           float tan_fovx, float tan_fovy, float focal_x, float focal_y, float kernel_size,
                           F3dgRec* rec, float2* means2D, float* depths, unsigned* sort_keys, uint2* rects, float4* bbox, float4* cull, float4* conic, int* radii,
                           unsigned* tiles, unsigned char* clamped, int save_aux, int tile_cull, F3dgHeaderInit init, uint2* chunk_boxes)
{
    const int grid_x = (W + F3DG_TILE - 1) / F3DG_TILE, grid_y = (H + F3DG_TILE - 1) / F3DG_TILE;
    const dim3 grid((P + F3DG_BLOCK - 1) / F3DG_BLOCK, V, 1);
#define F3DG_LAUNCH_PRE(AUX) F3DG_KLAUNCH((preprocess_kernel<AUX>), grid, dim3(F3DG_BLOCK), 0, s, P, D, M, views_per_set > 0 ? views_per_set : V, means3D, scales, \
                       scale_modifier, rotations, opacities, shs, cov3D_precomp, colors_precomp, v2g_precomp, viewmatrix, projmatrix,                  \
                       cam_pos, W, H, grid_x, grid_y, tan_fovx, tan_fovy, focal_x, focal_y, kernel_size, rec, means2D,                                  \
                       depths, sort_keys, rects, bbox, cull, conic, radii, tiles, clamped, tile_cull,                                                   \
                       1.0 / (double)focal_x, 1.0 / (double)focal_y, init, chunk_boxes)
    if (save_aux) F3DG_LAUNCH_PRE(true); else F3DG_LAUNCH_PRE(false);
#undef F3DG_LAUNCH_PRE
    F3DG_HIP_CHECK(hipGetLastError());
    return F3DG_OK;
}

extern "C" int f3dg_mark_visible(void* stream, int P, const float* means3D, const float* viewmatrix,
                                 const float* projmatrix, uint8_t* present)
{
    (void)projmatrix;
    if (P < 0 || (P > 0 && (!means3D || !viewmatrix || !present))) return F3DG_ERR_BAD_ARG;
    if (P == 0) return F3DG_OK;
    F3DG_KLAUNCH(mark_visible_kernel, dim3((P + 255) / 256), dim3(256), 0, (hipStream_t)stream, P, means3D,
                       viewmatrix, present);
    F3DG_HIP_CHECK(hipGetLastError());
    return F3DG_OK;
}
```

Before: 30300 views/s.

## Replace four-pass per-view depth radix sort with range-bucketed scatter plus per-bucket local sort

Preprocess now computes the per-view depth key range with wave and block reductions plus global atomics. The per-view depth sort uses that range to split keys into 255 linear buckets in a single histogram/scan/scatter pass. A new finish kernel then sorts each bucket in shared memory or in chunks, with only as many 8-bit passes as the bucket's key span needs. This replaces four global radix passes and the separate min/max range kernel, cutting global memory traffic and kernel launches. The cost is a memset, extra atomics in preprocess, and load imbalance when keys cluster in a few buckets.

Result: slower. 27430 views/s (-9.5%).

```diff
diff --git a/f3d-gaus_amd/csrc/f3dg_api.hip b/f3d-gaus_amd/csrc/f3dg_api.hip
--- a/f3d-gaus_amd/csrc/f3dg_api.hip
+++ b/f3d-gaus_amd/csrc/f3dg_api.hip
@@ -257,7 +257,7 @@
     L.vals[0] = take(C * 4);
     L.vals[1] = take(C * 4);
     L.segtab_minmax = (unsigned)((size_t)2 * (V + 1) + (size_t)8 * (V / 8 + 2));
-    L.segtab = take(((size_t)L.segtab_minmax + (size_t)2 * V + 2 * gsort_blocks) * sizeof(unsigned));
+    L.segtab = take(((size_t)L.segtab_minmax + (size_t)2 * V) * sizeof(unsigned));
     L.hist = take((size_t)256 * hist_blocks * sizeof(unsigned));
     L.ranges = take((size_t)V * T * sizeof(uint2));
     L.final_T = take((size_t)V * 4 * HW * sizeof(float));
@@ -301,6 +301,8 @@
                  const float* cam_pos, float tan_fovx, float tan_fovy, float focal_x, float focal_y, float kernel_size,
                  int* radii_used, int save_aux, int need_box, int tile_cull, ProfCall* prof, F3dgHeaderInit init, int small = 0)
 {
+    unsigned* key_range = small ? nullptr : reinterpret_cast<unsigned*>(ws + L.segtab) + L.segtab_minmax;
+    if (key_range) F3DG_HIP_CHECK(hipMemsetAsync(key_range, 0, sizeof(unsigned) * 2 * (size_t)n_views, s));
     int rc = f3dg_launch_preprocess(s, n_views, views_per_set, P, D, M, means3D, scales, scale_modifier, rotations, opacities, shs,
                                     cov3D_precomp, colors_precomp, view2gaussian_precomp, viewmatrix, projmatrix,
                                     cam_pos, W, H, tan_fovx, tan_fovy, focal_x, focal_y, kernel_size,
@@ -312,7 +314,7 @@
                                     reinterpret_cast<float4*>(ws + L.conic), radii_used,
                                     reinterpret_cast<unsigned*>(ws + L.tiles),
                                     reinterpret_cast<unsigned char*>(ws + L.clamped), save_aux, tile_cull, init,
-                                    small ? reinterpret_cast<uint2*>(ws + L.small_boxes) : nullptr);
+                                    small ? reinterpret_cast<uint2*>(ws + L.small_boxes) : nullptr, key_range);
     if (rc != F3DG_OK) return rc;
     prof_mark(prof, ST_PREPROCESS, s);
     rc = small ? f3dg_launch_small_bin(s, n_views, P, W, H, L, ws) : f3dg_launch_binning(s, n_views, P, W, H, L, ws, save_aux);
diff --git a/f3d-gaus_amd/csrc/f3dg_binning.hip b/f3d-gaus_amd/csrc/f3dg_binning.hip
--- a/f3d-gaus_amd/csrc/f3dg_binning.hip
+++ b/f3d-gaus_amd/csrc/f3dg_binning.hip
@@ -1,4 +1,5 @@
 #include "f3dg_common.h"
+#include "f3dg_depth_bucket.h"
 
 namespace {
 
@@ -139,16 +140,19 @@
     u32 mask = 255u;
     __device__ __forceinline__ u32 operator()(u32 k) const { return (k >> shift) & mask; }
 };
-struct CompactDigit {
-    u32 kbase;
-    __device__ __forceinline__ u32 operator()(u32 k) const { const u32 d = (k - kbase) >> 16; return d < 255u ? d : 255u; }
+struct BucketDigit {
+    u32 kmin, mlo, mhi;
+    __device__ __forceinline__ u32 operator()(u32 k) const
+    {
+        const u32 x = k - kmin;
+        return k == 0xFFFFFFFFu ? 255u : __umulhi(x, mlo) + x * mhi;
+    }
 };
 
-template <typename K, typename DIGIT, bool MINMAX = false>
+template <typename K, typename DIGIT>
 __device__ __forceinline__ void hist_chunk(const K* __restrict__ keys, const SegChunk& ck, const DIGIT digit, u32* __restrict__ hist,
-                                           u32 (*h)[256], u32* __restrict__ minmax = nullptr)
-{
-    u32 kmin = 0xFFFFFFFFu, kmax = 0u;
+                                           u32 (*h)[256])
+{
 #pragma unroll
     for (int w = 0; w < F3DG_BLOCK / 64; w++) h[w][threadIdx.x] = 0;
     __syncthreads();
@@ -161,30 +165,10 @@
     for (u64 a = (g0 & ~(u64)(VEC - 1)) + (u64)threadIdx.x * VEC; a < g1; a += (u64)F3DG_BLOCK * VEC) {
         const KV w = *reinterpret_cast<const KV*>(keys + a);
 #pragma unroll
-        for (int q = 0; q < VEC; q++) {
-            if (a + q >= g0 && a + q < g1) {
-                const u32 key = (u32)w[q];
-                atomicAdd(&hw[digit(key)], 1u);
-                if (MINMAX && key != 0xFFFFFFFFu) { kmin = key < kmin ? key : kmin; kmax = key > kmax ? key : kmax; }
-            }
-        }
-    }
-    __shared__ u32 wmm[2][F3DG_BLOCK / 64];
-    if (MINMAX) {
-#pragma unroll
-        for (int off = 32; off > 0; off >>= 1) {
-            const u32 a = __shfl_down(kmin, off, 64), b = __shfl_down(kmax, off, 64);
-            kmin = a < kmin ? a : kmin; kmax = b > kmax ? b : kmax;
-        }
-        if ((threadIdx.x & 63) == 0) { wmm[0][threadIdx.x >> 6] = kmin; wmm[1][threadIdx.x >> 6] = kmax; }
-    }
-    __syncthreads();
-    if (MINMAX && threadIdx.x == 0) {
-        u32 a = wmm[0][0], b = wmm[1][0];
-#pragma unroll
-        for (int w = 1; w < F3DG_BLOCK / 64; w++) { a = wmm[0][w] < a ? wmm[0][w] : a; b = wmm[1][w] > b ? wmm[1][w] : b; }
-        minmax[0] = a; minmax[1] = b;
-    }
+        for (int q = 0; q < VEC; q++)
+            if (a + q >= g0 && a + q < g1) atomicAdd(&hw[digit((u32)w[q])], 1u);
+    }
+    __syncthreads();
     hist[ck.obase + (u64)threadIdx.x * ck.cps + ck.c] = h[0][threadIdx.x] + h[1][threadIdx.x] + h[2][threadIdx.x] + h[3][threadIdx.x];
 }
 
@@ -293,37 +277,24 @@
     return ck;
 }
 
-__device__ __forceinline__ bool gsort_compact(const u32* __restrict__ minmax, u32 view, u32& kbase)
-{
-    const u32 kmin = minmax[2 * view], kmax = minmax[2 * view + 1];
-    kbase = kmin & 0xFFFF0000u;
-    return kmin <= kmax && ((kmax - kbase) >> 24) == 0u;
-}
-
-template <int PASS>
-__global__ void __launch_bounds__(F3DG_BLOCK)
-gsort_hist_kernel(const u32* __restrict__ keys, u32 seg_len, u32 cps, u32* __restrict__ hist, const u32* __restrict__ minmax,
-                  u32* __restrict__ chunk_minmax)
+__device__ __forceinline__ BucketDigit view_buckets(const u32* __restrict__ krange, u32 view, u32* bk)
+{
+    if (threadIdx.x == 0) {
+        const u32 kmin = ~krange[2 * view], kmax = krange[2 * view + 1];
+        const u64 m = f3dg_depth_bucket_mul(kmin, kmax);
+        bk[0] = kmin; bk[1] = (u32)m; bk[2] = (u32)(m >> 32);
+    }
+    __syncthreads();
+    return BucketDigit{bk[0], bk[1], bk[2]};
+}
+
+__global__ void __launch_bounds__(F3DG_BLOCK)
+gsort_hist_kernel(const u32* __restrict__ keys, u32 seg_len, u32 cps, u32* __restrict__ hist, const u32* __restrict__ krange)
 {
     __shared__ u32 h[F3DG_BLOCK / 64][256];
+    __shared__ u32 bk[3];
     const SegChunk ck = fixed_chunk(seg_len, cps);
-    if constexpr (PASS == 0) {
-        hist_chunk<u32, ShiftDigit>(keys, ck, ShiftDigit{0}, hist, h);
-    } else if constexpr (PASS == 1) {
-        hist_chunk<u32, ShiftDigit, true>(keys, ck, ShiftDigit{8}, hist, h, chunk_minmax + 2 * ((size_t)ck.seg * cps + ck.c));
-    } else {
-        u32 kbase;
-        const bool compact = gsort_compact(minmax, ck.seg, kbase);
-        if (!compact) {
-            hist_chunk<u32, ShiftDigit>(keys, ck, ShiftDigit{8 * PASS}, hist, h);
-        } else if constexpr (PASS == 2) {
-            hist_chunk<u32, CompactDigit>(keys, ck, CompactDigit{kbase}, hist, h);
-        } else {
-            const u64 base = (u64)ck.c * F3DG_SORT_CHUNK;
-            const u32 in_chunk = (u32)((ck.n - base) < (u64)F3DG_SORT_CHUNK ? (ck.n - base) : (u64)F3DG_SORT_CHUNK);
-            hist[ck.obase + (u64)threadIdx.x * ck.cps + ck.c] = threadIdx.x == 0 ? in_chunk : 0u;
-        }
-    }
+    hist_chunk<u32, BucketDigit>(keys, ck, view_buckets(krange, ck.seg, bk), hist, h);
 }
 
 __global__ void __launch_bounds__(1024)
@@ -358,42 +329,200 @@
     }
 }
 
-__global__ void __launch_bounds__(64)
-gsort_range_kernel(u32 cps, const u32* __restrict__ chunk_minmax, u32* __restrict__ minmax)
-{
-    u32 kmin = 0xFFFFFFFFu, kmax = 0u;
-    for (u32 c = threadIdx.x; c < cps; c += 64) {
-        const u32 a = chunk_minmax[2 * ((size_t)blockIdx.x * cps + c)], b = chunk_minmax[2 * ((size_t)blockIdx.x * cps + c) + 1];
-        kmin = a < kmin ? a : kmin; kmax = b > kmax ? b : kmax;
-    }
-#pragma unroll
-    for (int off = 32; off > 0; off >>= 1) {
-        const u32 a = __shfl_down(kmin, off, 64), b = __shfl_down(kmax, off, 64);
-        kmin = a < kmin ? a : kmin; kmax = b > kmax ? b : kmax;
-    }
-    if (threadIdx.x == 0) { minmax[2 * blockIdx.x] = kmin; minmax[2 * blockIdx.x + 1] = kmax; }
-}
-
-template <int PASS>
-__global__ void __launch_bounds__(F3DG_BLOCK)
-gsort_scatter_kernel(const u32* __restrict__ keys_in, const u32* __restrict__ vals_in, u32* __restrict__ keys_out,
-                     u32* __restrict__ vals_out, u32 seg_len, u32 cps, const u32* __restrict__ offsets, const u32* __restrict__ minmax)
+__global__ void __launch_bounds__(F3DG_BLOCK)
+gsort_scatter_kernel(const u32* __restrict__ keys_in, u32* __restrict__ keys_out, u32* __restrict__ vals_out, u32 seg_len, u32 cps,
+                     const u32* __restrict__ offsets, const u32* __restrict__ krange)
 {
     __shared__ ScatterShared sh;
     __shared__ u32 skey[F3DG_SORT_CHUNK];
+    __shared__ u32 bk[3];
     const SegChunk ck = fixed_chunk(seg_len, cps);
-    if constexpr (PASS == 0) {
-        scatter_chunk<u32, true, ShiftDigit>(keys_in, vals_in, keys_out, vals_out, ck, ShiftDigit{0}, offsets, sh, skey);
-    } else if constexpr (PASS == 1) {
-        scatter_chunk<u32, false, ShiftDigit>(keys_in, vals_in, keys_out, vals_out, ck, ShiftDigit{8}, offsets, sh, skey);
-    } else {
-        u32 kbase;
-        const bool compact = gsort_compact(minmax, ck.seg, kbase);
-        if (!compact)
-            scatter_chunk<u32, false, ShiftDigit>(keys_in, vals_in, PASS == 3 ? (u32*)nullptr : keys_out, vals_out, ck, ShiftDigit{8 * PASS}, offsets, sh, skey);
-        else if constexpr (PASS == 2)
-            scatter_chunk<u32, false, CompactDigit>(keys_in, vals_in, (u32*)nullptr, vals_out, ck, CompactDigit{kbase}, offsets, sh, skey);
-    }
+    scatter_chunk<u32, true, BucketDigit>(keys_in, nullptr, keys_out, vals_out, ck, view_buckets(krange, ck.seg, bk), offsets, sh, skey);
+}
+
+#define F3DG_FINISH_CAP F3DG_SORT_CHUNK
+struct FinishShared {
+    u32 cnt[F3DG_BLOCK / 64][256];
+    u32 lbase[256];
+    u32 tot[256];
+    u32 run[256];
+    u32 wtot[F3DG_BLOCK / 64];
+    u32 red[2][F3DG_BLOCK / 64];
+    u32 skey[F3DG_FINISH_CAP];
+    u32 sval[F3DG_FINISH_CAP];
+};
+
+__device__ __forceinline__ u32 finish_scan256(u32 v, u32* wtot)
+{
+    const u32 lane = threadIdx.x & 63u, wave = threadIdx.x >> 6;
+    u32 x = v;
+#pragma unroll
+    for (int off = 1; off < 64; off <<= 1) {
+        const u32 y = __shfl_up(x, off, 64);
+        if (lane >= (u32)off) x += y;
+    }
+    if (lane == 63u) wtot[wave] = x;
+    __syncthreads();
+    u32 excl = x - v;
+    for (u32 w = 0; w < wave; w++) excl += wtot[w];
+    return excl;
+}
+
+__device__ __forceinline__ void finish_minmax(u32& kmn, u32& kmx, u32 (*red)[F3DG_BLOCK / 64])
+{
+#pragma unroll
+    for (int off = 32; off > 0; off >>= 1) {
+        const u32 a = __shfl_xor(kmn, off, 64), b = __shfl_xor(kmx, off, 64);
+        kmn = a < kmn ? a : kmn; kmx = b > kmx ? b : kmx;
+    }
+    if ((threadIdx.x & 63u) == 0u) { red[0][threadIdx.x >> 6] = kmn; red[1][threadIdx.x >> 6] = kmx; }
+    __syncthreads();
+#pragma unroll
+    for (int w = 0; w < F3DG_BLOCK / 64; w++) { kmn = red[0][w] < kmn ? red[0][w] : kmn; kmx = red[1][w] > kmx ? red[1][w] : kmx; }
+}
+
+__device__ __forceinline__ void finish_rank(const u32 (&key)[F3DG_SORT_ITEMS], u32 (&slot)[F3DG_SORT_ITEMS], u32 rounds, u32 n, u32 sub,
+                                            int shift, FinishShared& sh)
+{
+    const u32 lane = threadIdx.x & 63u, wave = threadIdx.x >> 6;
+    const u32 i0 = wave * 64u * rounds + lane;
+    const u64 lane_lt = ((u64)1 << lane) - 1;
+#pragma unroll
+    for (int w = 0; w < F3DG_BLOCK / 64; w++) sh.cnt[w][threadIdx.x] = 0;
+    __syncthreads();
+#pragma unroll
+    for (int r = 0; r < F3DG_SORT_ITEMS; r++) {
+        if ((u32)r < rounds) {
+            const bool valid = i0 + 64u * r < n;
+            const u32 d = ((key[r] - sub) >> shift) & 255u;
+            u64 diff = 0;
+#pragma unroll
+            for (int b = 0; b < 8; b++) {
+                const u32 own = (u32)((int)(d << (31 - b)) >> 31);
+                const u64 bal = __ballot(own != 0u);
+                diff |= bal ^ (((u64)own << 32) | own);
+            }
+            const u64 same = __ballot(valid) & ~diff;
+            const u32 below = (u32)__popcll(same & lane_lt);
+            const u32 prev = sh.cnt[wave][d];
+            slot[r] = prev + below;
+            __builtin_amdgcn_wave_barrier();
+            if (valid && below == 0) sh.cnt[wave][d] = prev + (u32)__popcll(same);
+            __builtin_amdgcn_wave_barrier();
+        }
+    }
+    __syncthreads();
+    {
+        const u32 d = threadIdx.x;
+        const u32 c0 = sh.cnt[0][d], c1 = sh.cnt[1][d], c2 = sh.cnt[2][d], c3 = sh.cnt[3][d];
+        const u32 tot = c0 + c1 + c2 + c3;
+        const u32 excl = finish_scan256(tot, sh.wtot);
+        sh.lbase[d] = excl;
+        sh.tot[d] = tot;
+        sh.cnt[0][d] = excl;
+        sh.cnt[1][d] = excl + c0;
+        sh.cnt[2][d] = excl + c0 + c1;
+        sh.cnt[3][d] = excl + c0 + c1 + c2;
+    }
+    __syncthreads();
+#pragma unroll
+    for (int r = 0; r < F3DG_SORT_ITEMS; r++)
+        if ((u32)r < rounds) slot[r] += sh.cnt[wave][((key[r] - sub) >> shift) & 255u];
+}
+
+__global__ void __launch_bounds__(F3DG_BLOCK)
+gsort_finish_kernel(u32* gk0, u32* gk1, u32* perm, u32* gv1, u32 seg_len, u32 cps, const u32* __restrict__ offsets)
+{
+    __shared__ FinishShared sh;
+    u32 view, d;
+    f3dg_xcd_map(blockIdx.x, gridDim.x / 256u, 256u, view, d);
+    const u64 ob = (u64)view * 256u * cps;
+    const u32 lo = offsets[ob + (u64)d * cps];
+    const u32 hi = d < 255u ? offsets[ob + (u64)(d + 1u) * cps] : (view + 1u) * seg_len;
+    const u32 n = hi - lo;
+    const u32 lane = threadIdx.x & 63u, wave = threadIdx.x >> 6;
+    if (d == 255u || n <= 1u) {
+        for (u32 i = threadIdx.x; i < n; i += F3DG_BLOCK) perm[lo + i] = gv1[lo + i];
+        return;
+    }
+    u32 key[F3DG_SORT_ITEMS], val[F3DG_SORT_ITEMS], slot[F3DG_SORT_ITEMS];
+    u32 kmn = 0xFFFFFFFFu, kmx = 0u;
+    if (n <= (u32)F3DG_FINISH_CAP) {
+        const u32 rounds = (n + F3DG_BLOCK - 1) / F3DG_BLOCK;
+        const u32 i0 = wave * 64u * rounds + lane;
+#pragma unroll
+        for (int r = 0; r < F3DG_SORT_ITEMS; r++) {
+            const u32 i = i0 + 64u * r;
+            const bool valid = (u32)r < rounds && i < n;
+            key[r] = valid ? gk1[lo + i] : 0u;
+            val[r] = valid ? gv1[lo + i] : 0u;
+            if (valid) { kmn = key[r] < kmn ? key[r] : kmn; kmx = key[r] > kmx ? key[r] : kmx; }
+        }
+        finish_minmax(kmn, kmx, sh.red);
+        const u32 range = kmx - kmn;
+        const int passes = range == 0u ? 0 : (32 - __clz((int)range) + 7) / 8;
+        for (int p = 0; p < passes; p++) {
+            finish_rank(key, slot, rounds, n, kmn, 8 * p, sh);
+#pragma unroll
+            for (int r = 0; r < F3DG_SORT_ITEMS; r++)
+                if ((u32)r < rounds && i0 + 64u * r < n) { sh.skey[slot[r]] = key[r]; sh.sval[slot[r]] = val[r]; }
+            __syncthreads();
+#pragma unroll
+            for (int r = 0; r < F3DG_SORT_ITEMS; r++)
+                if ((u32)r < rounds && i0 + 64u * r < n) { key[r] = sh.skey[i0 + 64u * r]; val[r] = sh.sval[i0 + 64u * r]; }
+        }
+#pragma unroll
+        for (int r = 0; r < F3DG_SORT_ITEMS; r++)
+            if ((u32)r < rounds && i0 + 64u * r < n) perm[lo + i0 + 64u * r] = val[r];
+        return;
+    }
+    for (u32 i = threadIdx.x; i < n; i += F3DG_BLOCK) {
+        const u32 k = gk1[lo + i];
+        kmn = k < kmn ? k : kmn; kmx = k > kmx ? k : kmx;
+    }
+    finish_minmax(kmn, kmx, sh.red);
+    const u32 range = kmx - kmn;
+    const int passes = range == 0u ? 0 : (32 - __clz((int)range) + 7) / 8;
+    u32 *sk = gk1, *sv = gv1, *dk = gk0, *dv = perm;
+    for (int p = 0; p < passes; p++) {
+        const int shift = 8 * p;
+        sh.run[threadIdx.x] = 0u;
+        __syncthreads();
+        for (u32 i = threadIdx.x; i < n; i += F3DG_BLOCK) atomicAdd(&sh.run[((sk[lo + i] - kmn) >> shift) & 255u], 1u);
+        __syncthreads();
+        sh.run[threadIdx.x] = finish_scan256(sh.run[threadIdx.x], sh.wtot);
+        __syncthreads();
+        for (u32 c0 = 0; c0 < n; c0 += (u32)F3DG_FINISH_CAP) {
+            const u32 nc = n - c0 < (u32)F3DG_FINISH_CAP ? n - c0 : (u32)F3DG_FINISH_CAP;
+            const u32 rounds = (nc + F3DG_BLOCK - 1) / F3DG_BLOCK;
+            const u32 i0 = wave * 64u * rounds + lane;
+#pragma unroll
+            for (int r = 0; r < F3DG_SORT_ITEMS; r++) {
+                const u32 i = i0 + 64u * r;
+                const bool valid = (u32)r < rounds && i < nc;
+                key[r] = valid ? sk[lo + c0 + i] : 0u;
+                val[r] = valid ? sv[lo + c0 + i] : 0u;
+            }
+            finish_rank(key, slot, rounds, nc, kmn, shift, sh);
+#pragma unroll
+            for (int r = 0; r < F3DG_SORT_ITEMS; r++) {
+                if ((u32)r < rounds && i0 + 64u * r < nc) {
+                    const u32 dg = ((key[r] - kmn) >> shift) & 255u;
+                    const u32 pos = lo + sh.run[dg] + (slot[r] - sh.lbase[dg]);
+                    if (p + 1 < passes) dk[pos] = key[r];
+                    dv[pos] = val[r];
+                }
+            }
+            __syncthreads();
+            sh.run[threadIdx.x] += sh.tot[threadIdx.x];
+        }
+        __threadfence();
+        __syncthreads();
+        u32* t = sk; sk = dk; dk = t;
+        t = sv; sv = dv; dv = t;
+    }
+    if (sv != perm)
+        for (u32 i = threadIdx.x; i < n; i += F3DG_BLOCK) perm[lo + i] = sv[lo + i];
 }
 
 __global__ void __launch_bounds__(512)
@@ -507,18 +636,14 @@
 }
 
 __global__ void __launch_bounds__(F3DG_BLOCK)
-gsort_gather_rects_kernel(int P, u32* __restrict__ gv0, u32* __restrict__ gv1, const u32* __restrict__ minmax,
-                          const uint2* __restrict__ rects, u32* __restrict__ tiles_sorted, u32* __restrict__ rx)
+gsort_gather_rects_kernel(int P, const u32* __restrict__ perm, const uint2* __restrict__ rects, u32* __restrict__ tiles_sorted,
+                          u32* __restrict__ rx, u32* __restrict__ ry)
 {
     constexpr int ITEMS = 4;
     unsigned view, chunk;
     const unsigned cpv = (unsigned)((P + F3DG_BLOCK * ITEMS - 1) / (F3DG_BLOCK * ITEMS));
     f3dg_xcd_map(blockIdx.x, gridDim.x / cpv, cpv, view, chunk);
     const size_t vb = (size_t)view * P;
-    u32 kbase;
-    const bool pass2 = gsort_compact(minmax, view, kbase);
-    const u32* perm = pass2 ? gv1 : gv0;
-    u32* ry = pass2 ? gv0 : gv1;
     const int k0 = (int)(chunk * F3DG_BLOCK * ITEMS + threadIdx.x);
     u32 id[ITEMS];
     uint2 r[ITEMS];
@@ -541,9 +666,8 @@
 #define F3DG_DUP_CAP 3072
 template <typename G>
 __global__ void __launch_bounds__(F3DG_BLOCK)
-duplicate_sorted_kernel(int P, int tile_bits, int grid_x, const u32* __restrict__ gv0, const u32* __restrict__ gv1,
-                        const u32* __restrict__ minmax, const u32* __restrict__ rx,
-                        const u32* __restrict__ offsets_sorted,
+duplicate_sorted_kernel(int P, int tile_bits, int grid_x, const u32* __restrict__ perm, const u32* __restrict__ rx,
+                        const u32* __restrict__ ry, const u32* __restrict__ offsets_sorted,
                         const F3dgHeader* __restrict__ hdr, G* __restrict__ kgrp, u32* __restrict__ vals)
 {
     __shared__ G sk[F3DG_DUP_CAP];
@@ -551,10 +675,6 @@
     if (hdr->overflow) return;
     const int k = blockIdx.x * F3DG_BLOCK + threadIdx.x;
     const int v = blockIdx.y;
-    u32 kbase;
-    const bool pass2 = gsort_compact(minmax, (u32)v, kbase);
-    const u32* perm = pass2 ? gv1 : gv0;
-    const u32* ry = pass2 ? gv0 : gv1;
     const size_t first = (size_t)v * P + (size_t)blockIdx.x * F3DG_BLOCK;
     const int in_block = min(F3DG_BLOCK, P - (int)(blockIdx.x * F3DG_BLOCK));
     const u32 base = first == 0 ? 0u : offsets_sorted[first - 1];
@@ -697,34 +817,28 @@
 
     const u32 cps = (u32)((P + F3DG_SORT_CHUNK - 1) / F3DG_SORT_CHUNK);
     const u32 gblocks = (u32)V * cps;
-    u32* minmax = reinterpret_cast<u32*>(ws + L.segtab) + L.segtab_minmax;
-    u32* chunk_minmax = minmax + 2 * (size_t)V;
-    const bool view_scan = cps <= 64;
-#define F3DG_GSORT_PASS(PASS, IN, OUT)                                                                                                     \
-    F3DG_KLAUNCH((gsort_hist_kernel<PASS>), dim3(gblocks), dim3(F3DG_BLOCK), 0, s, gk[IN], (u32)P, cps, hist, minmax, chunk_minmax); \
-    if (view_scan)                                                                                                                         \
-        F3DG_KLAUNCH(gsort_scan_kernel, dim3(V), dim3(1024), 0, s, 256u * cps, (u32)P, hist);                                       \
-    else {                                                                                                                                 \
-        rc = f3dg_launch_scan_inclusive(s, hist, hist, (unsigned long long)256 * gblocks, scan_tmp, L.scan_tmp_elems, 1, nullptr);        \
-        if (rc != F3DG_OK) return rc;                                                                                                      \
-    }                                                                                                                                      \
-    F3DG_KLAUNCH((gsort_scatter_kernel<PASS>), dim3(gblocks), dim3(F3DG_BLOCK), 0, s, gk[IN], gv[IN], gk[OUT], gv[OUT], (u32)P, cps, hist, minmax)
-    F3DG_GSORT_PASS(0, 0, 1);
-    F3DG_GSORT_PASS(1, 1, 0);
-    F3DG_KLAUNCH(gsort_range_kernel, dim3(V), dim3(64), 0, s, cps, chunk_minmax, minmax);
-    F3DG_GSORT_PASS(2, 0, 1);
-    F3DG_GSORT_PASS(3, 1, 0);
-#undef F3DG_GSORT_PASS
+    const u32* krange = reinterpret_cast<const u32*>(ws + L.segtab) + L.segtab_minmax;
+    F3DG_KLAUNCH(gsort_hist_kernel, dim3(gblocks), dim3(F3DG_BLOCK), 0, s, gk[0], (u32)P, cps, hist, krange);
+    if (cps <= 64)
+        F3DG_KLAUNCH(gsort_scan_kernel, dim3(V), dim3(1024), 0, s, 256u * cps, (u32)P, hist);
+    else {
+        rc = f3dg_launch_scan_inclusive(s, hist, hist, (unsigned long long)256 * gblocks, scan_tmp, L.scan_tmp_elems, 1, nullptr);
+        if (rc != F3DG_OK) return rc;
+    }
+    F3DG_KLAUNCH(gsort_scatter_kernel, dim3(gblocks), dim3(F3DG_BLOCK), 0, s, gk[0], gk[1], gv[1], (u32)P, cps, hist, krange);
+    F3DG_KLAUNCH(gsort_finish_kernel, dim3((u32)V * 256u), dim3(F3DG_BLOCK), 0, s, gk[0], gk[1], gv[0], gv[1], (u32)P, cps, hist);
+    const u32* perm = gv[0];
     u32* offsets_sorted = gk[1];
     u32* rx = gk[0];
-
-    F3DG_KLAUNCH(gsort_gather_rects_kernel, dim3((unsigned)V * (unsigned)((P + 4 * F3DG_BLOCK - 1) / (4 * F3DG_BLOCK))), dim3(F3DG_BLOCK), 0, s, P, gv[0], gv[1], minmax,
-                           reinterpret_cast<const uint2*>(ws + L.rects), offsets_sorted, rx);
+    u32* ry = gv[1];
+
+    F3DG_KLAUNCH(gsort_gather_rects_kernel, dim3((unsigned)V * (unsigned)((P + 4 * F3DG_BLOCK - 1) / (4 * F3DG_BLOCK))), dim3(F3DG_BLOCK), 0, s, P, perm,
+                           reinterpret_cast<const uint2*>(ws + L.rects), offsets_sorted, rx, ry);
     rc = f3dg_launch_scan_inclusive(s, offsets_sorted, offsets_sorted, (unsigned long long)VP, scan_tmp, L.scan_tmp_elems, 0, hdr);
     if (rc != F3DG_OK) return rc;
     const int passes = f3dg_sort_passes(V, T);
     int src = passes & 1;
-    F3DG_KLAUNCH((duplicate_sorted_kernel<G>), pgrid, dim3(F3DG_BLOCK), 0, s, P, tile_bits, grid_x, gv[0], gv[1], minmax, rx, offsets_sorted, hdr,
+    F3DG_KLAUNCH((duplicate_sorted_kernel<G>), pgrid, dim3(F3DG_BLOCK), 0, s, P, tile_bits, grid_x, perm, rx, ry, offsets_sorted, hdr,
                        kgrp[src], vals[src]);
 
     if (passes > 0) {
diff --git a/f3d-gaus_amd/csrc/f3dg_common.h b/f3d-gaus_amd/csrc/f3dg_common.h
--- a/f3d-gaus_amd/csrc/f3dg_common.h
+++ b/f3d-gaus_amd/csrc/f3dg_common.h
@@ -145,7 +145,8 @@
                            float tan_fovx, float tan_fovy, float focal_x, float focal_y, float kernel_size,
                            F3dgRec* rec, float2* means2D, float* depths, unsigned* sort_keys, uint2* rects, float4* bbox , float4* cull, float4* conic,
                            int* radii, unsigned* tiles, unsigned char* clamped, int save_aux, int tile_cull, F3dgHeaderInit init,
-                           uint2* chunk_boxes = nullptr );
+                           uint2* chunk_boxes = nullptr ,
+                           unsigned* key_range = nullptr );
 
 #define F3DG_SMALL_CAP 4096
 inline bool f3dg_small_shape(int P, int W, int H, int V)
diff --git a/f3d-gaus_amd/csrc/f3dg_depth_bucket.h b/f3d-gaus_amd/csrc/f3dg_depth_bucket.h
--- /dev/null
+++ b/f3d-gaus_amd/csrc/f3dg_depth_bucket.h
@@ -0,0 +1,24 @@
+#pragma once
+#include <stdint.h>
+
+#if defined(__HIPCC__) || defined(__CUDACC__)
+#define F3DG_HD __host__ __device__ __forceinline__
+#else
+#define F3DG_HD inline
+#endif
+
+#define F3DG_DEPTH_BUCKETS 255u
+
+F3DG_HD uint64_t f3dg_depth_bucket_mul(uint32_t kmin, uint32_t kmax)
+{
+    if (kmin > kmax) return 0ull;
+    const uint64_t R = (uint64_t)(kmax - kmin) + 1ull;
+    return ((uint64_t)F3DG_DEPTH_BUCKETS << 32) / R;
+}
+
+F3DG_HD uint32_t f3dg_depth_bucket(uint32_t key, uint32_t kmin, uint64_t mul)
+{
+    if (key == 0xFFFFFFFFu) return 255u;
+    const uint32_t x = key - kmin;
+    return (uint32_t)(((uint64_t)x * (uint32_t)mul) >> 32) + x * (uint32_t)(mul >> 32);
+}
diff --git a/f3d-gaus_amd/csrc/f3dg_preprocess.hip b/f3d-gaus_amd/csrc/f3dg_preprocess.hip
--- a/f3d-gaus_amd/csrc/f3dg_preprocess.hip
+++ b/f3d-gaus_amd/csrc/f3dg_preprocess.hip
@@ -162,8 +162,12 @@
                   float4* __restrict__ conic_out,
                   int* __restrict__ radii, unsigned* __restrict__ tiles_touched,
                   unsigned char* __restrict__ clamped, int tile_cull,
-                  double inv_focal_x, double inv_focal_y, F3dgHeaderInit init, uint2* __restrict__ chunk_boxes)
-{
+                  double inv_focal_x, double inv_focal_y, F3dgHeaderInit init, uint2* __restrict__ chunk_boxes,
+                  unsigned* __restrict__ key_range)
+{
+    __shared__ unsigned s_range[2], s_waves_done;
+    if (threadIdx.x < 3) (threadIdx.x < 2 ? s_range[threadIdx.x] : s_waves_done) = 0u;
+    __syncthreads();
     if (init.hdr != nullptr && blockIdx.x == 0 && blockIdx.y == 0 && threadIdx.x < 64) {
         reinterpret_cast<unsigned*>(init.hdr)[threadIdx.x] = 0;
         if (threadIdx.x == 0) {
@@ -450,7 +454,30 @@
         }
         if ((threadIdx.x & 63u) == 0u) chunk_boxes[(size_t)v * ((P + 63) / 64) + (g >> 6)] = bx;
     }
-    sort_keys[idx] = my_tiles ? __float_as_uint(depth) : 0xFFFFFFFFu;
+    const unsigned sort_key = my_tiles ? __float_as_uint(depth) : 0xFFFFFFFFu;
+    sort_keys[idx] = sort_key;
+    if (key_range) {
+        unsigned a = my_tiles ? ~sort_key : 0u, b = my_tiles ? sort_key : 0u;
+        if (__ballot(true) == ~0ull) {
+#pragma unroll
+            for (int off = 32; off > 0; off >>= 1) {
+                const unsigned a2 = __shfl_xor(a, off, 64), b2 = __shfl_xor(b, off, 64);
+                a = a2 > a ? a2 : a; b = b2 > b ? b2 : b;
+            }
+            if ((threadIdx.x & 63u) != 0u) a = b = 0u;
+        }
+        if (a) atomicMax(&s_range[0], a);
+        if (b) atomicMax(&s_range[1], b);
+        const int live = P - (int)(blockIdx.x * F3DG_BLOCK);
+        const unsigned waves = live >= F3DG_BLOCK ? F3DG_BLOCK / 64 : (unsigned)((live + 63) / 64);
+        if ((threadIdx.x & 63u) == 0u &&
+            __hip_atomic_fetch_add(&s_waves_done, 1u, __ATOMIC_ACQ_REL, __HIP_MEMORY_SCOPE_WORKGROUP) == waves - 1u) {
+            const unsigned ra = __hip_atomic_load(&s_range[0], __ATOMIC_RELAXED, __HIP_MEMORY_SCOPE_WORKGROUP);
+            const unsigned rb = __hip_atomic_load(&s_range[1], __ATOMIC_RELAXED, __HIP_MEMORY_SCOPE_WORKGROUP);
+            if (ra > __hip_atomic_load(&key_range[2 * v], __ATOMIC_RELAXED, __HIP_MEMORY_SCOPE_AGENT)) atomicMax(&key_range[2 * v], ra);
+            if (rb > __hip_atomic_load(&key_range[2 * v + 1], __ATOMIC_RELAXED, __HIP_MEMORY_SCOPE_AGENT)) atomicMax(&key_range[2 * v + 1], rb);
+        }
+    }
     if (bbox_out) bbox_out[idx] = box;
     if (SAVE_AUX || my_tiles != 0u) {
         r3.w = cec;
@@ -485,7 +512,8 @@
                            const float* viewmatrix, const float* projmatrix, const float* cam_pos, int W, int H,
                            float tan_fovx, float tan_fovy, float focal_x, float focal_y, float kernel_size,
                            F3dgRec* rec, float2* means2D, float* depths, unsigned* sort_keys, uint2* rects, float4* bbox, float4* cull, float4* conic, int* radii,
-                           unsigned* tiles, unsigned char* clamped, int save_aux, int tile_cull, F3dgHeaderInit init, uint2* chunk_boxes)
+                           unsigned* tiles, unsigned char* clamped, int save_aux, int tile_cull, F3dgHeaderInit init, uint2* chunk_boxes,
+                           unsigned* key_range)
 {
     const int grid_x = (W + F3DG_TILE - 1) / F3DG_TILE, grid_y = (H + F3DG_TILE - 1) / F3DG_TILE;
     const dim3 grid((P + F3DG_BLOCK - 1) / F3DG_BLOCK, V, 1);
@@ -493,7 +521,7 @@
                        scale_modifier, rotations, opacities, shs, cov3D_precomp, colors_precomp, v2g_precomp, viewmatrix, projmatrix,                  \
                        cam_pos, W, H, grid_x, grid_y, tan_fovx, tan_fovy, focal_x, focal_y, kernel_size, rec, means2D,                                  \
                        depths, sort_keys, rects, bbox, cull, conic, radii, tiles, clamped, tile_cull,                                                   \
-                       1.0 / (double)focal_x, 1.0 / (double)focal_y, init, chunk_boxes)
+                       1.0 / (double)focal_x, 1.0 / (double)focal_y, init, chunk_boxes, key_range)
     if (save_aux) F3DG_LAUNCH_PRE(true); else F3DG_LAUNCH_PRE(false);
 #undef F3DG_LAUNCH_PRE
     F3DG_HIP_CHECK(hipGetLastError());
```
